# OpenDriveLab/ViDAR

Hardware: AMD Instinct MI355X
Metric: train samples/sec (6-cam->BEV step) (higher is better)
Workload: dtype f32

## Files before the change

### include/vidar_hip.h

```cpp
#ifndef VIDAR_HIP_H_
#define VIDAR_HIP_H_

#include <stddef.h>
#include <stdint.h>

#ifdef __cplusplus
extern "C" {
#endif

#define VIDAR_ERR_BAD_ARG (-22)

int vidar_abi_version(void);
int vidar_marker(int id, void* stream);

int vidar_set_deterministic(int on);
int vidar_get_deterministic(void);

int vidar_dvr_max_d(void);

int vidar_dvr_render_forward_f32(const float* sigma, const float* origin, const float* points,
                                 const float* tindex, float* pred_dist ,
                                 float* gt_dist , int N, int M, int T, int TO, int Z, int Y,
                                 int X, int train_phase, void* stream);

int vidar_dvr_render_f32(const float* sigma, const float* origin, const float* points,
                         const float* tindex, float* pred_dist, float* gt_dist, float* grad_sigma,
                         int N, int M, int T, int TO, int Z, int Y, int X, int loss_type,
                         void* stream);

int vidar_dvr_init_f32(const float* points, const float* tindex, float* occupancy, int N, int M,
                       int T, int Z, int Y, int X, void* stream);

int vidar_dvxlr_max_d(void);


int vidar_dvr_set_sort_min_waves(int min_waves);
int vidar_dvr_set_traversal(int mode);
int vidar_dvxlr_set_pad_mode(int mode);

int vidar_dvxlr_render_f32(const float* sigma, const float* origin, const float* points,
                           const float* tindex, float* pred_dist, float* gt_dist, float* dd_dsigma,
                           float* indices, int N, int M, int T, int TO, int Z, int Y, int X,
                           void* stream);

size_t vidar_dvxlr_get_grad_sigma_workspace_bytes(int N, int T, int Z, int Y, int X, int volumes );
int vidar_dvxlr_get_grad_sigma_f32(const float* elementwise_mult ,
                                   const float* indices , const float* tindex,
                                   float* grad_sigma , int N, int M, int L, int T,
                                   int Z, int Y, int X, void* workspace, size_t workspace_bytes,
                                   void* stream);

int vidar_dvxlr2_render_f32(const float* sigma, const float* origin, const float* points,
                            const float* tindex, const float* sigma_regul, float* pred_dist,
                            float* gt_dist, float* dd_dsigma, float* indices, float* ray_pred,
                            float* indicator, int N, int M, int T, int TO, int Z, int Y, int X,
                            void* stream);

int vidar_dvxlr2_get_grad_sigma_f32(const float* elementwise_mult, const float* indices,
                                    const float* tindex, const float* indicator,
                                    const float* grad_ray_pred, float* grad_sigma,
                                    float* grad_sigma_regul, int N, int M, int L, int T, int Z, int Y,
                                    int X, void* workspace, size_t workspace_bytes, void* stream);

size_t vidar_knn1_d3_workspace_bytes(int N, int P1);
int vidar_knn1_d3_fwd(const float* p1, const float* p2, const int64_t* lengths1,
                      const int64_t* lengths2, int64_t* idx, float* dist2, void* workspace, int N,
                      int P1, int P2, void* stream);
int vidar_knn1_d3_bwd(const float* p1, const float* p2, const int64_t* lengths1,
                      const int64_t* lengths2, const int64_t* idx, const float* grad_dist2,
                      float* grad_p1, float* grad_p2, int N, int P1, int P2, void* stream);
int vidar_knn1_d3_bwd_workspace_bytes(int N, int P2, int64_t* bytes);
int vidar_knn1_d3_bwd_ws(const float* p1, const float* p2, const int64_t* lengths1,
                         const int64_t* lengths2, const int64_t* idx, const float* grad_dist2,
                         float* grad_p1, float* grad_p2, int N, int P1, int P2, void* workspace,
                         size_t workspace_bytes, void* stream);

int vidar_msda_fwd_f32(const float* value, const int64_t* spatial_shapes,
                       const int64_t* level_start_index, const float* sampling_loc,
                       const float* attn_weight, float* out, int B, int Nv, int H, int C, int Nq,
                       int L, int P, void* stream);
size_t vidar_msda_bwd_workspace_bytes(int B, int Nv, int H, int Nq, int L, int P);
int vidar_msda_set_item_order(int head_major);
int vidar_msda_bwd_f32(const float* value, const int64_t* spatial_shapes,
                       const int64_t* level_start_index, const float* sampling_loc,
                       const float* attn_weight, const float* grad_out, float* grad_value,
                       float* grad_sampling_loc, float* grad_attn_weight, int B, int Nv, int H, int C,
                       int Nq, int L, int P, void* workspace, size_t workspace_bytes, void* stream);

int vidar_msda_fused_fwd_f32(const float* value, const int64_t* spatial_shapes,
                             const int64_t* level_start_index, const float* off_raw, const float* logit_raw,
                             const float* ref, float* loc_out, float* w_out, float* out, int bs, int Qn, int Nv,
                             int H, int C, int Nq, int L, int P, int R, int mode, int merge_queue, void* stream);
int vidar_msda_fused_bwd_f32(const float* value, const int64_t* spatial_shapes,
                             const int64_t* level_start_index, const float* sampling_loc,
                             const float* attn_weight, const float* grad_out, float* grad_value,
                             float* grad_off_raw, float* grad_logit_raw, int bs, int Qn, int Nv, int H, int C,
                             int Nq, int L, int P, int merge_queue, void* workspace, size_t workspace_bytes, void* stream);

int vidar_drop_add_ln_fwd_f32(const float* x, const float* residual, const float* gamma, const float* beta, float* y,
                              float* sum_out, float* mean_out, float* rstd_out, int64_t rows, int C, float p, float eps,
                              uint32_t seed, void* stream);
int vidar_drop_add_ln_bwd_f32(const float* grad_y, const float* sum_in, const float* gamma, const float* mean_in,
                              const float* rstd_in, float* grad_x, float* grad_residual, float* grad_gamma,
                              float* grad_beta, void* workspace, int64_t rows, int C, float p, uint32_t seed,
                              void* stream);
size_t vidar_drop_add_ln_bwd_workspace_bytes(int64_t rows);

int vidar_relu_drop_fwd_f32(const float* x, float* y, int64_t n, float p, uint32_t seed, void* stream);
int vidar_relu_drop_bwd_f32(const float* grad_y, const float* y, float* grad_x, int64_t n, float p, void* stream);

int vidar_colsum_f32(const float* x, float* out, int64_t rows, int cols, void* stream);

int vidar_sca_plan_f32(const float* ref_3d, const float* lidar2img, float* ref_cam, uint8_t* bev_mask,
                       float* count, int64_t* idx, uint8_t* valid, int32_t* lens, int32_t* slot_of,
                       const float* pc_range, float img_h, float img_w, int F, int B, int N, int Q, int D,
                       void* stream);
int vidar_sca_rows_f32(const float* src, const int64_t* idx, const uint8_t* valid, const float* count, float* dst,
                       int B, int N, int S, int stride, int Q, int C, void* stream);
int vidar_sca_combine_f32(const float* src, const int32_t* slot_of, const float* count, float* dst, int B, int N,
                          int S, int Q, int C, void* stream);

size_t vidar_latent_render_bwd_workspace_bytes(int bs, int H, int W, int Z, int maps );
int vidar_latent_render_prob_fwd_f32(const float* occ, float* path_prob, int bs, int H, int W, int Z,
                                     int grid_num, float step, int act, void* stream);
int vidar_latent_render_prob_bwd_f32(const float* occ, const float* grad_path_prob, float* grad_occ,
                                     int bs, int H, int W, int Z, int grid_num, float step, int act,
                                     void* workspace, size_t workspace_bytes, void* stream);
int vidar_latent_render_gather_fwd_f32(const float* path_prob, const float* lora_a, float* feat,
                                       float* msum, int bs, int H, int W, int Z, int grid_num,
                                       float step, float eps, void* stream);
int vidar_latent_render_gather_bwd_f32(const float* path_prob, const float* lora_a, const float* feat,
                                       const float* msum, const float* grad_feat,
                                       float* grad_path_prob, float* grad_lora_a, int bs, int H,
                                       int W, int Z, int grid_num, float step, float eps,
                                       void* workspace, size_t workspace_bytes, void* stream);
int vidar_latent_render_gather_grouped_fwd_f32(const float* path_prob, const float* lora_a, float* feat, float* msum,
                                               int bs, int H, int W, int Z, int A, int grid_num, float step,
                                               float eps, void* stream);
int vidar_latent_render_gather_grouped_bwd_f32(const float* path_prob, const float* lora_a, const float* feat,
                                               const float* msum, const float* grad_feat, float* grad_path_prob,
                                               float* grad_lora_a, int bs, int H, int W, int Z, int A, int grid_num,
                                               float step, float eps, void* workspace, size_t workspace_bytes,
                                               void* stream);

size_t vidar_ray_bwd_workspace_bytes(int F, int Z, int Y, int X);
int vidar_ray_ce_fwd_f32(const float* sigma, const float* origin, const float* gt_pts,
                         const float* tindex, float* ce, float* lse, float* valid, int F, int R,
                         int Z, int Y, int X, int K, float step, void* stream);
int vidar_ray_ce_bwd_f32(const float* sigma, const float* origin, const float* gt_pts,
                         const float* tindex, const float* lse, const float* grad_ce,
                         float* grad_sigma, int F, int R, int Z, int Y, int X, int K, float step,
                         void* workspace, size_t workspace_bytes, void* stream);
int vidar_ray_gumbel_fwd_f32(const float* sigma, const float* origin, const float* pts,
                             const float* tindex, const float* noise , float* dist,
                             float* aux , int F, int R, int Z, int Y, int X, int K,
                             float step, void* stream);
int vidar_ray_gumbel_bwd_f32(const float* sigma, const float* origin, const float* pts,
                             const float* tindex, const float* aux, const float* grad_dist,
                             float* grad_sigma, int F, int R, int Z, int Y, int X, int K, float step,
                             void* workspace, size_t workspace_bytes, void* stream);
int vidar_ray_argmax_f32(const float* sigma, const float* origin, const float* pts,
                         const float* tindex, float* pred_dist, float* gt_dist, int F, int R, int Z,
                         int Y, int X, int K, float step, void* stream);
int vidar_ray_dist_fwd_f32(const float* sigma, const float* origin, const float* gt_pts,
                           const float* tindex, const float* noise , float* dist,
                           float* gt_len, float* aux , float* valid, int F, int R, int Z,
                           int Y, int X, int K, float step, void* stream);
int vidar_ray_dist_bwd_f32(const float* sigma, const float* origin, const float* gt_pts,
                           const float* tindex, const float* aux, const float* grad_dist,
                           float* grad_sigma, int F, int R, int Z, int Y, int X, int K, float step,
                           void* workspace, size_t workspace_bytes, void* stream);
int vidar_ray_max_k(void);
int vidar_ray_force_streamed(int on);

#define VIDAR_GEMM_F32 0
#define VIDAR_GEMM_BF16X3 1
#define VIDAR_GEMM_K_MAJOR 0
#define VIDAR_GEMM_MN_MAJOR 1
int vidar_gemm_f32(const float* A, int64_t lda, int a_layout, const float* B, int64_t ldb, int b_layout, float* C,
                   int64_t ldc, int M, int N, int K, int batch, int64_t strideA, int64_t strideB, int64_t strideC,
                   const float* scale, const float* shift, int vec_axis, const float* residual, int64_t ldr,
                   int64_t strideR, int relu, int precision, int reduce, float* a_rowsum, void* workspace,
                   size_t workspace_bytes, void* stream);
int vidar_gemm_splits(int M, int N, int K, int batch, int precision, int reduce);
size_t vidar_gemm_workspace_bytes(int M, int N, int K, int batch, int precision, int reduce);
int vidar_gemm_set_variant(int variant);

int vidar_dcn_set_variant(int variant);
int vidar_dcn_im2col_f32(const float* x, const float* offset, const float* mask, float* cols, int N,
                         int C, int H, int W, int Ho, int Wo, int kh, int kw, int stride, int pad,
                         int dil, void* stream);
int vidar_dcn_col2im_det_workspace_bytes(int N, int C, int H, int W, int64_t* bytes);
int vidar_dcn_col2im_f32(const float* grad_cols, const float* x, const float* offset,
                         const float* mask, float* grad_x, float* grad_offset, float* grad_mask,
                         int N, int C, int H, int W, int Ho, int Wo, int kh, int kw, int stride,
                         int pad, int dil, void* workspace, size_t workspace_bytes, void* stream);
size_t vidar_dcn_col2im_workspace_bytes(int N, int H, int W, int Ho, int Wo, int kh, int kw);

size_t vidar_conv3x3_few_workspace_bytes(int C);
int vidar_conv3x3_few_f32(const float* x, const float* weight, const float* bias, float* out, int N, int C, int H, int W,
                          int Cout, void* workspace, size_t workspace_bytes, void* stream);

int vidar_affine_act_fwd_f32(const float* x, const float* scale, const float* shift,
                             const float* residual, float* y, int N, int C, int HW, int relu,
                             void* stream);
int vidar_stem_bn_relu_pool_f32(const float* x, const float* scale, const float* shift, float* y, int N, int C,
                                int H, int W, void* stream);
int vidar_affine_act_bwd_f32(const float* grad_y, const float* y, const float* scale, float* grad_x,
                             float* grad_residual, int N, int C, int HW, int relu, void* stream);

int vidar_dcnv3_set_variant(int variant);
int vidar_dcnv3_forward_f32(const float* input, const float* offset, const float* mask, float* out, int N, int H, int W,
                            int kh, int kw, int stride_h, int stride_w, int pad_h, int pad_w, int dil_h, int dil_w,
                            int group, int group_channels, float offset_scale, void* stream);
size_t vidar_dcnv3_backward_workspace_bytes(int N, int H, int W, int kh, int kw, int stride_h, int stride_w, int pad_h,
                                            int pad_w, int dil_h, int dil_w, int group, int group_channels);
int vidar_dcnv3_backward_f32(const float* input, const float* offset, const float* mask, const float* grad_out,
                             float* grad_input, float* grad_offset, float* grad_mask, int N, int H, int W, int kh, int kw,
                             int stride_h, int stride_w, int pad_h, int pad_w, int dil_h, int dil_w, int group,
                             int group_channels, float offset_scale, void* workspace, size_t workspace_bytes, void* stream);

int vidar_det_match_cost_f32(const float* cls, const float* box, const float* gt_box_norm, const int32_t* gt_label,
                             const int32_t* gt_start, float* cost, float alpha, float gamma, float cls_weight,
                             float reg_weight, int NL, int B, int Q, int C, int total_g, void* stream);
size_t vidar_det_loss_workspace_bytes(int NL, int B, int Q);
int vidar_det_loss_fwd_f32(const float* cls, const float* box, const int32_t* labels, const int32_t* matched_gt,
                           const float* gt_box_norm, const int32_t* gt_start, const float* code_weights, float* sums,
                           float alpha, float gamma, int NL, int B, int Q, int C, int total_g, void* workspace,
                           size_t workspace_bytes, void* stream);
int vidar_det_loss_bwd_f32(const float* cls, const float* box, const int32_t* labels, const int32_t* matched_gt,
                           const float* gt_box_norm, const int32_t* gt_start, const float* code_weights,
                           const float* grad_sums, float* grad_cls, float* grad_box, float alpha, float gamma, int NL,
                           int B, int Q, int C, int total_g, void* stream);

#define VIDAR_IMG_PHOTO_FLOATS 12
int vidar_img_photometric_u8(const uint8_t* src, const float* photo, uint8_t* dst, int n, int H, int W, void* stream);
int vidar_img_photometric_f32(const uint8_t* src, const float* photo, float* dst, int n, int H, int W, void* stream);
size_t vidar_img_resample_workspace_bytes(int n, int crop_h, int out_w);
int vidar_img_resample_u8(const uint8_t* src, uint8_t* dst, int n, int H, int W, int crop_x, int crop_y, int crop_w,
                          int crop_h, int out_w, int out_h, const int32_t* tab_x, int ksize_x, const int32_t* tab_y,
                          int ksize_y, int flip, void* workspace, size_t workspace_bytes, void* stream);
int vidar_img_normalise_f32(const uint8_t* src, const float* photo, float* dst, int n, int H, int W, int out_h, int out_w,
                            int Hp, int Wp, const float* mean, const float* stdv, int to_rgb, void* stream);

#ifdef __cplusplus
}
#endif
#endif
```

### vidar_amd/_lib.py

```python
from __future__ import annotations

import ctypes
import os
from pathlib import Path

_PKG = Path(__file__).resolve().parent
LIB_PATH = _PKG / "libvidar_hip.so"
_lib = None
BAD_ARG = -22


class VidarHipError(RuntimeError):
    pass


def lib() -> ctypes.CDLL:
    global _lib
    if _lib is None:
        import torch
        if not LIB_PATH.exists():
            raise VidarHipError(
                f"{LIB_PATH} not found: build it with `python -m vidar_amd.build` "
                f"(or __graft_entry__.build()); vidar_amd has no CPU fallback")
        _lib = declare(ctypes.CDLL(str(LIB_PATH)))
        dcn = os.environ.get("VIDAR_DCN_VARIANT")
        if dcn is not None:
            _lib.vidar_dcn_set_variant(int(dcn))
        v3 = os.environ.get("VIDAR_DCNV3_VARIANT")
        if v3 is not None:
            _lib.vidar_dcnv3_set_variant(int(v3))
        order = os.environ.get("VIDAR_MSDA_ITEM_ORDER")
        if order is not None:
            _lib.vidar_msda_set_item_order(int(order))
    return _lib


_KIND = {"p": ctypes.c_void_p, "i": ctypes.c_int, "l": ctypes.c_int64, "z": ctypes.c_size_t, "f": ctypes.c_float,
         "u": ctypes.c_uint32}
_ABI = {
    "vidar_abi_version": "i",
    "vidar_marker": "i i p",
    "vidar_set_deterministic": "i i",
    "vidar_get_deterministic": "i",
    "vidar_dvr_max_d": "i",
    "vidar_dvr_render_forward_f32": "i 6p 8i p",
    "vidar_dvr_render_f32": "i 7p 8i p",
    "vidar_dvr_init_f32": "i 3p 6i p",
    "vidar_dvxlr_max_d": "i",
    "vidar_dvr_set_sort_min_waves": "i i",
    "vidar_dvr_set_traversal": "i i",
    "vidar_dvxlr_set_pad_mode": "i i",
    "vidar_dvxlr_render_f32": "i 8p 7i p",
    "vidar_dvxlr_get_grad_sigma_workspace_bytes": "z 6i",
    "vidar_dvxlr_get_grad_sigma_f32": "i 4p 7i p z p",
    "vidar_dvxlr2_render_f32": "i 11p 7i p",
    "vidar_dvxlr2_get_grad_sigma_f32": "i 7p 7i p z p",
    "vidar_knn1_d3_workspace_bytes": "z 2i",
    "vidar_knn1_d3_fwd": "i 7p 3i p",
    "vidar_knn1_d3_bwd": "i 8p 3i p",
    "vidar_knn1_d3_bwd_workspace_bytes": "i 2i p",
    "vidar_knn1_d3_bwd_ws": "i 8p 3i p z p",
    "vidar_msda_fwd_f32": "i 6p 7i p",
    "vidar_msda_bwd_workspace_bytes": "z 6i",
    "vidar_msda_set_item_order": "i i",
    "vidar_msda_bwd_f32": "i 9p 7i p z p",
    "vidar_msda_fused_fwd_f32": "i 9p 11i p",
    "vidar_msda_fused_bwd_f32": "i 9p 9i p z p",
    "vidar_drop_add_ln_fwd_f32": "i 8p l i 2f u p",
    "vidar_drop_add_ln_bwd_f32": "i 10p l i f u p",
    "vidar_drop_add_ln_bwd_workspace_bytes": "z l",
    "vidar_relu_drop_fwd_f32": "i 2p l f u p",
    "vidar_relu_drop_bwd_f32": "i 3p l f p",
    "vidar_colsum_f32": "i 2p l i p",
    "vidar_sca_plan_f32": "i 10p 2f 5i p",
    "vidar_sca_rows_f32": "i 5p 6i p",
    "vidar_sca_combine_f32": "i 4p 5i p",
    "vidar_latent_render_bwd_workspace_bytes": "z 5i",
    "vidar_latent_render_prob_fwd_f32": "i 2p 5i f i p",
    "vidar_latent_render_prob_bwd_f32": "i 3p 5i f i p z p",
    "vidar_latent_render_gather_fwd_f32": "i 4p 5i 2f p",
    "vidar_latent_render_gather_bwd_f32": "i 7p 5i 2f p z p",
    "vidar_latent_render_gather_grouped_fwd_f32": "i 4p 6i 2f p",
    "vidar_latent_render_gather_grouped_bwd_f32": "i 7p 6i 2f p z p",
    "vidar_ray_bwd_workspace_bytes": "z 4i",
    "vidar_ray_ce_fwd_f32": "i 7p 6i f p",
    "vidar_ray_ce_bwd_f32": "i 7p 6i f p z p",
    "vidar_ray_gumbel_fwd_f32": "i 7p 6i f p",
    "vidar_ray_gumbel_bwd_f32": "i 7p 6i f p z p",
    "vidar_ray_argmax_f32": "i 6p 6i f p",
    "vidar_ray_dist_fwd_f32": "i 9p 6i f p",
    "vidar_ray_dist_bwd_f32": "i 7p 6i f p z p",
    "vidar_ray_max_k": "i",
    "vidar_ray_force_streamed": "i i",
    "vidar_gemm_f32": "i p l i p l i p l 4i 3l 2p i p 2l 3i 2p z p",
    "vidar_gemm_splits": "i 6i",
    "vidar_gemm_workspace_bytes": "z 6i",
    "vidar_gemm_set_variant": "i i",
    "vidar_dcn_set_variant": "i i",
    "vidar_dcn_im2col_f32": "i 4p 11i p",
    "vidar_dcn_col2im_f32": "i 7p 11i p z p",
    "vidar_dcn_col2im_workspace_bytes": "z 7i",
    "vidar_dcn_col2im_det_workspace_bytes": "i 4i p",
    "vidar_conv3x3_few_workspace_bytes": "z i",
    "vidar_conv3x3_few_f32": "i 4p 5i p z p",
    "vidar_affine_act_fwd_f32": "i 5p 4i p",
    "vidar_stem_bn_relu_pool_f32": "i 4p 4i p",
    "vidar_affine_act_bwd_f32": "i 5p 4i p",
    "vidar_dcnv3_set_variant": "i i",
    "vidar_dcnv3_forward_f32": "i 4p 13i f p",
    "vidar_dcnv3_backward_workspace_bytes": "z 13i",
    "vidar_dcnv3_backward_f32": "i 7p 13i f p z p",
    "vidar_det_match_cost_f32": "i 6p 4f 5i p",
    "vidar_det_loss_workspace_bytes": "z 3i",
    "vidar_det_loss_fwd_f32": "i 8p 2f 5i p z p",
    "vidar_det_loss_bwd_f32": "i 10p 2f 5i p",
    "vidar_img_photometric_u8": "i 3p 3i p",
    "vidar_img_photometric_f32": "i 3p 3i p",
    "vidar_img_resample_workspace_bytes": "z 3i",
    "vidar_img_resample_u8": "i 2p 9i p i p 2i p z p",
    "vidar_img_normalise_f32": "i 3p 7i 2p i p",
}


def signature(name):
    ret, *runs = _ABI[name].split()
    return _KIND[ret], [_KIND[r[-1]] for r in runs for _ in range(int(r[:-1] or 1))]


def declare(cdll):
    for name in _ABI:
        try:
            fn = getattr(cdll, name)
        except AttributeError:
            raise VidarHipError(f"{name} is not exported by {cdll._name}: rebuild the library") from None
        fn.restype, fn.argtypes = signature(name)
    return cdll


def check(rc: int, what: str):
    if rc == 0:
        return
    if rc == BAD_ARG:
        raise ValueError(f"{what}: invalid argument")
    raise VidarHipError(f"{what}: HIP error {rc}")


def ptr(t):
    return None if t is None else t.data_ptr()


def workspace(nbytes_fn, *dims, like):
    import torch
    n = nbytes_fn(*dims)
    if n == 0:
        return None, None, 0
    ws = torch.empty(n, dtype=torch.uint8, device=like.device)
    return ws, ptr(ws), n


def stream_of(t):
    import torch
    return torch.cuda.current_stream(t.device).cuda_stream


class OpTimer:
    def __init__(self):
        self.enabled = False
        self.records = {}

    def reset(self):
        self.records = {}

    class _Span:
        __slots__ = ("t", "name", "nbytes", "e0")

        def __init__(self, t, name, nbytes):
            self.t, self.name, self.nbytes = t, name, nbytes

        def __enter__(self):
            import torch
            self.e0 = torch.cuda.Event(enable_timing=True)
            self.e0.record()

        def __exit__(self, *exc):
            import torch
            e1 = torch.cuda.Event(enable_timing=True)
            e1.record()
            self.t.records.setdefault(self.name, []).append((self.e0, e1, self.nbytes))

    class _Null:
        def __enter__(self): return None
        def __exit__(self, *exc): return False

    _null = _Null()

    def span(self, name, nbytes=0):
        return OpTimer._Span(self, name, nbytes) if self.enabled else OpTimer._null

    def summary(self):
        import torch
        torch.cuda.synchronize()
        out = {}
        for name, recs in self.records.items():
            ms = [a.elapsed_time(b) for a, b, _ in recs]
            out[name] = dict(calls=len(ms), total_ms=sum(ms), avg_ms=sum(ms) / len(ms),
                             bytes_per_call=sum(r[2] for r in recs) / len(recs))
        return out


TIMER = OpTimer()
```

### vidar_amd/csrc/dcn.hip

```cpp
#include <hip/hip_runtime.h>
#include <stdint.h>

#include "vidar_hip.h"
#include "vidar_common.h"
#include "det_scatter.h"

namespace {

struct PlaneTile { int plane, tile; bool ok; };
__device__ __forceinline__ PlaneTile xcd_plane_tile(int L, int T, int planes) {
  const int xcd = L & 7, j = L >> 3;
  const int pl = (j / T) * 8 + xcd;
  return PlaneTile{pl, j - (j / T) * T, pl < planes};
}
inline unsigned xcd_plane_grid(int T, int planes) { return 8u * (unsigned)T * (unsigned)((planes + 7) / 8); }

struct Conv { int C, H, W, Ho, Wo, kh, kw, stride, pad, dil; };

struct Bil {
  int h0, w0;
  float lh, lw;
  bool in, t, b, l, r;
};

__device__ __forceinline__ Bil bil(float h, float w, int H, int W) {
  Bil q;
  q.in = h > -1.f && w > -1.f && h < H && w < W;
  q.h0 = (int)floorf(h); q.w0 = (int)floorf(w);
  q.lh = h - q.h0; q.lw = w - q.w0;
  q.t = q.h0 >= 0; q.b = q.h0 + 1 <= H - 1; q.l = q.w0 >= 0; q.r = q.w0 + 1 <= W - 1;
  return q;
}

struct Pos { float h, w; };
__device__ __forceinline__ Pos tap_pos(const Conv& g, int py, int px, int t, float oh, float ow) {
  const int i = t / g.kw, j = t - i * g.kw;
  return Pos{py * g.stride - g.pad + i * g.dil + oh, px * g.stride - g.pad + j * g.dil + ow};
}

template <class F>
__device__ __forceinline__ void for_corners(const Bil& q, int W, F f) {
  const float hh = 1.f - q.lh, hw = 1.f - q.lw;
  const int tl = q.h0 * W + q.w0;
  if (q.t && q.l) f(tl, hh * hw);
  if (q.t && q.r) f(tl + 1, hh * q.lw);
  if (q.b && q.l) f(tl + W, q.lh * hw);
  if (q.b && q.r) f(tl + W + 1, q.lh * q.lw);
}

constexpr int kMaxTaps = 9;

typedef float pair_t __attribute__((ext_vector_type(2), aligned(4)));

template <bool PAIR>
__device__ __forceinline__ pair_t load_pair(const void* p) {
  if constexpr (PAIR) return *reinterpret_cast<const pair_t*>(p);
  else return pair_t{*reinterpret_cast<const float*>(p), 0.f};
}

struct PairMap {
  int top, bot;
  bool same, left;
  __device__ __forceinline__ float e0(float cl, float cr) const { return same ? cl : (left ? cr : 0.f); }
  __device__ __forceinline__ float e1(float cl, float cr) const { return same ? cr : (left ? 0.f : cl); }
};

__device__ __forceinline__ PairMap pair_map(const Bil& q, int H, int W) {
  const int c0 = min(max(q.w0, 0), max(W - 2, 0));
  const int r0 = min(max(q.h0, 0), H - 1), r1 = min(max(q.h0 + 1, 0), H - 1);
  return PairMap{r0 * W + c0, r1 * W + c0, q.w0 == c0, q.w0 < c0};
}

constexpr int kCP = 16;
struct TapFoot { unsigned top, bot; float wt0, wt1, wb0, wb1; };

__device__ __forceinline__ TapFoot tap_foot(Pos s, float m, const Conv& g) {
  const Bil q = bil(s.h, s.w, g.H, g.W);
  const PairMap pm = pair_map(q, g.H, g.W);
  const float wl = (q.l ? 1.f - q.lw : 0.f), wr = (q.r ? q.lw : 0.f);
  const float a0 = pm.e0(wl, wr), a1 = pm.e1(wl, wr);
  const float ht = (q.t ? 1.f - q.lh : 0.f) * m, hb = (q.b ? q.lh : 0.f) * m;
  TapFoot f;
  f.top = (unsigned)pm.top * 4u; f.bot = (unsigned)pm.bot * 4u;
  f.wt0 = q.in ? ht * a0 : 0.f; f.wt1 = q.in ? ht * a1 : 0.f;
  f.wb0 = q.in ? hb * a0 : 0.f; f.wb1 = q.in ? hb * a1 : 0.f;
  return f;
}

template <bool PAIR>
__device__ __forceinline__ void im2col_body(const float* __restrict__ x, const float* __restrict__ offset,
                                            const float* __restrict__ mask, float* __restrict__ cols, const Conv& g, int nimg) {
  const int P = g.Ho * g.Wo, K = g.kh * g.kw;
  const int cgroups = (g.C + kCP - 1) / kCP;
  const PlaneTile pt = xcd_plane_tile(blockIdx.x, (P + 255) / 256, cgroups * nimg);
  if (!pt.ok) return;
  const int p = pt.tile * 256 + threadIdx.x;
  if (p >= P) return;
  const int n = pt.plane / cgroups, c0 = (pt.plane - n * cgroups) * kCP, nc = min(kCP, g.C - c0);
  const int py = p / g.Wo, px = p % g.Wo;
  const size_t plane = (size_t)g.H * g.W, KP = (size_t)K * P;
  const char* im = reinterpret_cast<const char*>(x + ((size_t)n * g.C + c0) * plane);
  float* out = cols + ((size_t)n * g.C + c0) * KP + p;
  const float* off_n = offset + (size_t)n * 2 * K * P + p;
  const float* msk_n = mask + (size_t)n * K * P + p;
  float oh = off_n[0], ow = off_n[P], m = msk_n[0];
  for (int t = 0; t < K; ++t) {
    const TapFoot f = tap_foot(tap_pos(g, py, px, t, oh, ow), m, g);
    pair_t a[kCP], b[kCP];
#pragma unroll
    for (int c = 0; c < kCP; ++c) {
      const char* pl = im + (size_t)(c < nc ? c : 0) * plane * 4;
      a[c] = load_pair<PAIR>(pl + f.top);
      b[c] = load_pair<PAIR>(pl + f.bot);
    }
    if (t + 1 < K) {
      oh = off_n[(size_t)(2 * t + 2) * P]; ow = off_n[(size_t)(2 * t + 3) * P]; m = msk_n[(size_t)(t + 1) * P];
    }
#pragma unroll
    for (int c = 0; c < kCP; ++c)
      if (c < nc) {
        const float v = f.wt0 * a[c].x + f.wt1 * a[c].y + f.wb0 * b[c].x + f.wb1 * b[c].y;
        __builtin_nontemporal_store(v, out + (size_t)c * KP + (size_t)t * P);
      }
  }
}

__global__ __launch_bounds__(256) void dcn_im2col_pair_kernel(
    const float* __restrict__ x, const float* __restrict__ offset, const float* __restrict__ mask,
    float* __restrict__ cols, Conv g, int nimg) {
  im2col_body<true>(x, offset, mask, cols, g, nimg);
}
__global__ __launch_bounds__(256) void dcn_im2col_kernel(
    const float* __restrict__ x, const float* __restrict__ offset, const float* __restrict__ mask,
    float* __restrict__ cols, Conv g, int nimg) {
  im2col_body<false>(x, offset, mask, cols, g, nimg);
}

constexpr int kCG = 8;
template <class Acc, class... AccParam>
__global__ __launch_bounds__(256) void dcn_col2im_kernel(const float* __restrict__ grad_cols, const float* __restrict__ offset,
                                                         const float* __restrict__ mask, float* __restrict__ grad_x, Conv g,
                                                         AccParam... acc_param) {
  Acc acc(grad_x, acc_param...);
  const int P = g.Ho * g.Wo, K = g.kh * g.kw;
  const int p = blockIdx.x * 256 + threadIdx.x;
  if constexpr (!Acc::kMeasureOnly) {
    if (p >= P) return;
  }
  const int n = blockIdx.z, c0 = blockIdx.y * kCG, nc = min(kCG, g.C - c0);
  const int py = p / g.Wo, px = p % g.Wo;
  const size_t plane = (size_t)g.H * g.W, KP = (size_t)K * P;
  float* gim = grad_x + ((size_t)n * g.C + c0) * plane;
  const float* gc = grad_cols + ((size_t)n * g.C + c0) * KP + p;
  for (int t = 0; t < K; ++t) {
    if constexpr (Acc::kMeasureOnly) {
      if (p >= P) break;
    }
    const size_t o = ((size_t)n * 2 * K + 2 * t) * P + p;
    const Pos s = tap_pos(g, py, px, t, offset[o], offset[o + P]);
    const Bil q = bil(s.h, s.w, g.H, g.W);
    if (!q.in) continue;
    const float m = mask[((size_t)n * K + t) * P + p];
    for (int c = 0; c < nc; ++c) {
      const float gv = gc[(size_t)c * KP + (size_t)t * P] * m;
      if (gv == 0.f) continue;
      for_corners(q, g.W, [&](int pix, float w) { acc.add(gim + (size_t)c * plane + pix, w * gv); });
    }
  }
  if constexpr (Acc::kMeasureOnly) acc.flush();
}

struct Entry { int src; float w; };

template <bool FILL>
__global__ __launch_bounds__(256) void dcn_revmap_kernel(const float* __restrict__ offset,
                                                         const float* __restrict__ mask, int* __restrict__ cursor,
                                                         Entry* __restrict__ rec, Conv g) {
  const int P = g.Ho * g.Wo, K = g.kh * g.kw, HW = g.H * g.W;
  const int p = blockIdx.x * 256 + threadIdx.x;
  if (p >= P) return;
  const int t = blockIdx.y, n = blockIdx.z;
  const int py = p / g.Wo, px = p % g.Wo;
  const size_t o = ((size_t)n * 2 * K + 2 * t) * P + p;
  const Pos s = tap_pos(g, py, px, t, offset[o], offset[o + P]);
  const Bil q = bil(s.h, s.w, g.H, g.W);
  if (!q.in) return;
  const float m = FILL ? mask[((size_t)n * K + t) * P + p] : 0.f;
  int* cur = cursor + ((size_t)n * K + t) * HW;
  const int src = t * P + p;
  for_corners(q, g.W, [&](int pix, float w) {
    if (FILL) rec[atomicAdd(cur + pix, 1)] = Entry{src, w * m};
    else atomicAdd(cur + pix, 1);
  });
}

__global__ __launch_bounds__(1024) void dcn_revmap_scan_kernel(int* __restrict__ cursor, int* __restrict__ first,
                                                               int HW, int per_image) {
  __shared__ int s_part[1024];
  const int n = blockIdx.x;
  int* cnt = cursor + (size_t)n * HW;
  int* fst = first + (size_t)n * HW;
  const int per = (HW + 1023) / 1024;
  const int r0 = min(HW, (int)threadIdx.x * per), r1 = min(HW, r0 + per);
  int sum = 0;
  for (int i = r0; i < r1; ++i) sum += cnt[i];
  s_part[threadIdx.x] = sum;
  __syncthreads();
  for (int d = 1; d < 1024; d <<= 1) {
    const int a = (int)threadIdx.x >= d ? s_part[threadIdx.x - d] : 0;
    __syncthreads();
    s_part[threadIdx.x] += a;
    __syncthreads();
  }
  int run = n * per_image + s_part[threadIdx.x] - sum;
  for (int i = r0; i < r1; ++i) { const int c = cnt[i]; fst[i] = run; cnt[i] = run; run += c; }
}

constexpr int kGC = 16;
__global__ __launch_bounds__(256) void dcn_col2im_gather_kernel(const float* __restrict__ grad_cols,
                                                                const int* __restrict__ first,
                                                                const int* __restrict__ last,
                                                                const Entry* __restrict__ rec,
                                                                float* __restrict__ grad_x, Conv g) {
  const int P = g.Ho * g.Wo, K = g.kh * g.kw, HW = g.H * g.W;
  const int pix = blockIdx.x * 256 + threadIdx.x;
  if (pix >= HW) return;
  const int n = blockIdx.z, c0 = blockIdx.y * kGC;
  float acc[kGC];
#pragma unroll
  for (int c = 0; c < kGC; ++c) acc[c] = 0.f;
  const size_t KP = (size_t)K * P;
  const float* gc = grad_cols + ((size_t)n * g.C + c0) * KP;
  const int nc = min(kGC, g.C - c0);
  for (int t = 0; t < K; ++t) {
    const size_t bin = ((size_t)n * K + t) * HW + pix;
    const int e0 = first[bin], e1 = last[bin];
    if (nc == kGC) {
      int e = e0;
      for (; e + 1 < e1; e += 2) {
        const Entry r0 = rec[e], r1 = rec[e + 1];
        float v0[kGC], v1[kGC];
#pragma unroll
        for (int c = 0; c < kGC; ++c) { v0[c] = gc[(size_t)c * KP + r0.src]; v1[c] = gc[(size_t)c * KP + r1.src]; }
#pragma unroll
        for (int c = 0; c < kGC; ++c) acc[c] += r0.w * v0[c] + r1.w * v1[c];
      }
      if (e < e1) {
        const Entry r = rec[e];
#pragma unroll
        for (int c = 0; c < kGC; ++c) acc[c] += r.w * gc[(size_t)c * KP + r.src];
      }
    } else {
      for (int e = e0; e < e1; ++e) {
        const Entry r = rec[e];
        for (int c = 0; c < nc; ++c) acc[c] += r.w * gc[(size_t)c * KP + r.src];
      }
    }
  }
  for (int c = 0; c < nc; ++c) grad_x[((size_t)n * g.C + c0 + c) * HW + pix] = acc[c];
}

#ifndef VIDAR_DCN_GRY
#define VIDAR_DCN_GRY 2
#endif
#ifndef VIDAR_DCN_GLC
#define VIDAR_DCN_GLC 8
#endif
constexpr int kGRY = VIDAR_DCN_GRY;
constexpr int kGTH = 8 * kGRY, kGTW = 32;
#ifndef VIDAR_DCN_GHALO
#define VIDAR_DCN_GHALO 5
#endif
constexpr int kGHalo = VIDAR_DCN_GHALO;
constexpr int kGWH = kGTH + 2 * kGHalo + 2;
constexpr int kGWW = kGTW + 2 * kGHalo + 2;
constexpr int kGWP = (kGWW + 3) / 4 * 4;
constexpr int kGWS = kGWH * kGWP;
constexpr int kGLC = VIDAR_DCN_GLC;
constexpr int kGPos = (kGWS + 255) / 256;

__global__ __launch_bounds__(256) void dcn_col2im_gather_lds_kernel(
    const float* __restrict__ grad_cols, const int* __restrict__ first, const int* __restrict__ last,
    const Entry* __restrict__ rec, float* __restrict__ grad_x, Conv g, int tiles_x, int tiles_y, int nimg, float inv_wo) {
  __shared__ __attribute__((aligned(16))) float s_gc[kGLC * kGWS];
  constexpr int K = 9;
  const int P = g.Ho * g.Wo, HW = g.H * g.W;
  const int cgroups = (g.C + kGLC - 1) / kGLC;
  const PlaneTile pt = xcd_plane_tile(blockIdx.x, tiles_x * tiles_y, cgroups * nimg);
  if (!pt.ok) return;
  const int tile = pt.tile, tyi = tile / tiles_x, txi = tile - tyi * tiles_x;
  const int n = pt.plane / cgroups, c0 = (pt.plane - n * cgroups) * kGLC, nc = min(kGLC, g.C - c0);
  const int ry = threadIdx.x / kGTW, rx = threadIdx.x % kGTW;
  const int dx = txi * kGTW + rx;
  const size_t KP = (size_t)K * P;
  const float* gc = grad_cols + ((size_t)n * g.C + c0) * KP;
  float acc[kGRY][kGLC];
#pragma unroll
  for (int k = 0; k < kGRY; ++k)
#pragma unroll
    for (int c = 0; c < kGLC; ++c) acc[k][c] = 0.f;
  for (int t = 0; t < K; ++t) {
    const int i = t / 3, j = t - i * 3;
    const int wy0 = tyi * kGTH + g.pad - i - kGHalo - 1, wx0 = txi * kGTW + g.pad - j - kGHalo - 1;
    const float* gct = gc + (size_t)t * P;
    __syncthreads();
    {
      const int wave = __builtin_amdgcn_readfirstlane((int)threadIdx.x >> 6);
#pragma unroll
      for (int k = 0; k < kGPos; ++k) {
        const int e = threadIdx.x + k * 256;
        const int r = e / kGWP, cc = e - r * kGWP;
        const int sy = wy0 + r, sx = wx0 + cc;
        const bool ok = e < kGWS && sy >= 0 && sy < g.Ho && sx >= 0 && sx < g.Wo && cc < kGWW;
        const int off = ok ? sy * g.Wo + sx : 0;
        if (ok) {
#pragma unroll
          for (int c = 0; c < kGLC; ++c)
            __builtin_amdgcn_global_load_lds((const __attribute__((address_space(1))) void*)(gct + (size_t)(c < nc ? c : 0) * KP + off),
                                             (__attribute__((address_space(3))) void*)(s_gc + c * kGWS + k * 256 + wave * 64), 4, 0, 0);
        }
      }
    }
    __syncthreads();
    if (dx >= g.W) continue;
#pragma unroll
    for (int k = 0; k < kGRY; ++k) {
      const int dy = tyi * kGTH + ry + 8 * k;
      if (dy >= g.H) continue;
      const size_t bin = ((size_t)n * K + t) * HW + dy * g.W + dx;
      const int e1 = last[bin];
      int e = first[bin];
      Entry nxt = e < e1 ? rec[e] : Entry{0, 0.f};
      while (e < e1) {
        const Entry r = nxt;
        ++e;
        if (e < e1) nxt = rec[e];
        const int p = r.src - t * P;
        const int py = (int)((p + 0.5f) * inv_wo), px = p - py * g.Wo;
        const int ly = py - wy0, lx = px - wx0;
        if (ly >= 0 && ly < kGWH && lx >= 0 && lx < kGWW) {
          const float* q = s_gc + ly * kGWP + lx;
#pragma unroll
          for (int c = 0; c < kGLC; ++c) acc[k][c] += r.w * q[c * kGWS];
        } else {
          for (int c = 0; c < nc; ++c) acc[k][c] += r.w * gct[(size_t)c * KP + p];
        }
      }
    }
  }
  if (dx < g.W) {
#pragma unroll
    for (int k = 0; k < kGRY; ++k) {
      const int dy = tyi * kGTH + ry + 8 * k;
      if (dy < g.H)
        for (int c = 0; c < nc; ++c) grad_x[((size_t)n * g.C + c0 + c) * HW + dy * g.W + dx] = acc[k][c];
    }
  }
}

int g_dcn_variant = 1;

template <bool PAIR>
__device__ __forceinline__ void col2im_coord_body(const float* __restrict__ grad_cols, const float* __restrict__ x,
                                                  const float* __restrict__ offset, const float* __restrict__ mask,
                                                  float* __restrict__ grad_offset, float* __restrict__ grad_mask,
                                                  const Conv& g) {
  const int P = g.Ho * g.Wo, K = g.kh * g.kw;
  const int p = blockIdx.x * 256 + threadIdx.x;
  if (p >= P) return;
  const int t = blockIdx.y, n = blockIdx.z;
  const int py = p / g.Wo, px = p % g.Wo;
  const size_t o = ((size_t)n * 2 * K + 2 * t) * P + p;
  const Pos s = tap_pos(g, py, px, t, offset[o], offset[o + P]);
  const float m = mask[((size_t)n * K + t) * P + p];
  const Bil q = bil(s.h, s.w, g.H, g.W);
  float gh = 0.f, gw = 0.f, gm = 0.f;
  if (q.in) {
    const float hh = 1.f - q.lh, hw = 1.f - q.lw;
    const PairMap pm = pair_map(q, g.H, g.W);
    const float tl = (q.t && q.l) ? 1.f : 0.f, tr = (q.t && q.r) ? 1.f : 0.f;
    const float bl = (q.b && q.l) ? 1.f : 0.f, br = (q.b && q.r) ? 1.f : 0.f;
    const float m_t0 = pm.e0(hh * hw * tl, hh * q.lw * tr), m_t1 = pm.e1(hh * hw * tl, hh * q.lw * tr);
    const float m_b0 = pm.e0(q.lh * hw * bl, q.lh * q.lw * br), m_b1 = pm.e1(q.lh * hw * bl, q.lh * q.lw * br);
    const float h_t0 = pm.e0(-hw * tl, -q.lw * tr), h_t1 = pm.e1(-hw * tl, -q.lw * tr);
    const float h_b0 = pm.e0(hw * bl, q.lw * br), h_b1 = pm.e1(hw * bl, q.lw * br);
    const float w_t0 = pm.e0(-hh * tl, hh * tr), w_t1 = pm.e1(-hh * tl, hh * tr);
    const float w_b0 = pm.e0(-q.lh * bl, q.lh * br), w_b1 = pm.e1(-q.lh * bl, q.lh * br);
    int c = 0;
    constexpr int kCB = 8;
    const unsigned top_b = (unsigned)pm.top * 4u, bot_b = (unsigned)pm.bot * 4u, p_b = (unsigned)p * 4u;
    const size_t plane_b = (size_t)g.H * g.W * 4, col_b = (size_t)K * P * 4;
    for (; c + kCB <= g.C; c += kCB) {
      const char* im0 = reinterpret_cast<const char*>(x) + ((size_t)n * g.C + c) * plane_b;
      const char* gc0 = reinterpret_cast<const char*>(grad_cols) + (((size_t)n * g.C + c) * K + t) * (size_t)P * 4;
      pair_t a[kCB], b[kCB];
      float gc[kCB];
#pragma unroll
      for (int u = 0; u < kCB; ++u) {
        gc[u] = *reinterpret_cast<const float*>(gc0 + u * col_b + p_b);
        a[u] = load_pair<PAIR>(im0 + u * plane_b + top_b);
        b[u] = load_pair<PAIR>(im0 + u * plane_b + bot_b);
      }
      __builtin_amdgcn_sched_barrier(0);
#pragma unroll
      for (int u = 0; u < kCB; ++u) {
        gm += gc[u] * (m_t0 * a[u].x + m_t1 * a[u].y + m_b0 * b[u].x + m_b1 * b[u].y);
        gh += gc[u] * (h_t0 * a[u].x + h_t1 * a[u].y + h_b0 * b[u].x + h_b1 * b[u].y);
        gw += gc[u] * (w_t0 * a[u].x + w_t1 * a[u].y + w_b0 * b[u].x + w_b1 * b[u].y);
      }
    }
    for (; c < g.C; ++c) {
      const float* im = x + ((size_t)n * g.C + c) * g.H * g.W;
      const float gc = grad_cols[(((size_t)n * g.C + c) * K + t) * P + p];
      const pair_t a = load_pair<PAIR>(im + pm.top), b = load_pair<PAIR>(im + pm.bot);
      gm += gc * (m_t0 * a.x + m_t1 * a.y + m_b0 * b.x + m_b1 * b.y);
      gh += gc * (h_t0 * a.x + h_t1 * a.y + h_b0 * b.x + h_b1 * b.y);
      gw += gc * (w_t0 * a.x + w_t1 * a.y + w_b0 * b.x + w_b1 * b.y);
    }
  }
  grad_offset[o] = gh * m;
  grad_offset[o + P] = gw * m;
  grad_mask[((size_t)n * K + t) * P + p] = gm;
}

__global__ __launch_bounds__(256) void dcn_col2im_coord_kernel(
    const float* __restrict__ grad_cols, const float* __restrict__ x, const float* __restrict__ offset,
    const float* __restrict__ mask, float* __restrict__ grad_offset, float* __restrict__ grad_mask, Conv g) {
  col2im_coord_body<true>(grad_cols, x, offset, mask, grad_offset, grad_mask, g);
}
__global__ __launch_bounds__(256) void dcn_col2im_coord_1col_kernel(
    const float* __restrict__ grad_cols, const float* __restrict__ x, const float* __restrict__ offset,
    const float* __restrict__ mask, float* __restrict__ grad_offset, float* __restrict__ grad_mask, Conv g) {
  col2im_coord_body<false>(grad_cols, x, offset, mask, grad_offset, grad_mask, g);
}

inline bool dcn_bad(int N, const Conv& g) {
  return N < 0 || g.C <= 0 || g.H <= 0 || g.W <= 0 || g.Ho <= 0 || g.Wo <= 0 || g.kh <= 0 ||
         g.kw <= 0 || g.stride <= 0 || g.dil <= 0 || g.pad < 0;
}

}

extern "C" {

int vidar_dcn_set_variant(int variant) {
  const int prev = g_dcn_variant;
  if (variant >= 0 && variant <= 1) g_dcn_variant = variant;
  return prev;
}

int vidar_dcn_im2col_f32(const float* x, const float* offset, const float* mask, float* cols, int N,
                         int C, int H, int W, int Ho, int Wo, int kh, int kw, int stride, int pad,
                         int dil, void* stream) {
  VIDAR_ENTER();
  Conv g{C, H, W, Ho, Wo, kh, kw, stride, pad, dil};
  if (dcn_bad(N, g)) return VIDAR_ERR_BAD_ARG;
  if (N == 0) return 0;
  if (kh * kw > kMaxTaps) return VIDAR_ERR_BAD_ARG;
  hipLaunchKernelGGL(W >= 2 ? dcn_im2col_pair_kernel : dcn_im2col_kernel,
                     dim3(xcd_plane_grid((Ho * Wo + 255) / 256, ((C + kCP - 1) / kCP) * N)), dim3(256), 0, (hipStream_t)stream,
                     x, offset, mask, cols, g, N);
  return vidar_last_error();
}

size_t vidar_dcn_col2im_workspace_bytes(int N, int H, int W, int Ho, int Wo, int kh, int kw) {
  if (N <= 0 || H <= 0 || W <= 0 || Ho <= 0 || Wo <= 0 || kh <= 0 || kw <= 0) return 0;
  const size_t hw = (size_t)N * kh * kw * H * W, ent = (size_t)N * kh * kw * Ho * Wo * 4;
  if (ent >= (1ull << 31)) return 0;
  return sizeof(int) * 2 * hw + sizeof(Entry) * ent;
}

int vidar_dcn_col2im_det_workspace_bytes(int N, int C, int H, int W, int64_t* bytes) {
  if (N < 0 || C < 0 || H < 0 || W < 0 || !bytes) return VIDAR_ERR_BAD_ARG;
  *bytes = (int64_t)det_workspace_bytes((size_t)N * C * H * W);
  return 0;
}

int vidar_dcn_col2im_f32(const float* grad_cols, const float* x, const float* offset,
                         const float* mask, float* grad_x, float* grad_offset, float* grad_mask,
                         int N, int C, int H, int W, int Ho, int Wo, int kh, int kw, int stride,
                         int pad, int dil, void* workspace, size_t workspace_bytes, void* stream) {
  VIDAR_ENTER();
  Conv g{C, H, W, Ho, Wo, kh, kw, stride, pad, dil};
  if (dcn_bad(N, g)) return VIDAR_ERR_BAD_ARG;
  hipStream_t s = (hipStream_t)stream;
  if (N == 0) return 0;
  if (kh * kw > kMaxTaps) return VIDAR_ERR_BAD_ARG;
  const int P = Ho * Wo, K = kh * kw, HW = H * W;
  if (det_mode()) {
    const dim3 grid((P + 255) / 256, (C + kCG - 1) / kCG, N);
    const int rc = det_scatter(
        grad_x, nullptr, (size_t)N * C * HW, 0, (uint64_t)N * C * K * P * 4, false, workspace, workspace_bytes, s,
        [&](uint32_t* word, uint32_t*) {
          hipLaunchKernelGGL((dcn_col2im_kernel<det::AccMeasure, det::AccMeasure::Param>), grid, dim3(256), 0, s, grad_cols, offset, mask, grad_x, g,
                             det::AccMeasure::Param{word});
        },
        [&](long long* acc, long long*, const uint32_t* word, const uint32_t*, int h) {
          hipLaunchKernelGGL((dcn_col2im_kernel<det::AccFixed, det::AccFixed::Param>), grid, dim3(256), 0, s, grad_cols, offset, mask, grad_x, g,
                             det::AccFixed::Param{acc, word, h});
        });
    if (rc != 0) return rc;
  } else if (workspace) {
    const size_t need = vidar_dcn_col2im_workspace_bytes(N, H, W, Ho, Wo, kh, kw);
    if (need == 0 || workspace_bytes < need) return VIDAR_ERR_BAD_ARG;
    int* cursor = (int*)workspace;
    int* first = cursor + (size_t)N * K * HW;
    Entry* rec = (Entry*)(first + (size_t)N * K * HW);
    hipError_t e = hipMemsetAsync(cursor, 0, sizeof(int) * (size_t)N * K * HW, s);
    if (e != hipSuccess) return (int)e;
    const dim3 rgrid((P + 255) / 256, K, N);
    hipLaunchKernelGGL(dcn_revmap_kernel<false>, rgrid, dim3(256), 0, s, offset, mask, cursor, rec, g);
    hipLaunchKernelGGL(dcn_revmap_scan_kernel, dim3(N * K), dim3(1024), 0, s, cursor, first, HW, P * 4);
    hipLaunchKernelGGL(dcn_revmap_kernel<true>, rgrid, dim3(256), 0, s, offset, mask, cursor, rec, g);
    if ((g_dcn_variant & 1) && kh == 3 && kw == 3 && stride == 1 && dil == 1 && Ho == H && Wo == W) {
      const int tiles_x = (W + kGTW - 1) / kGTW, tiles_y = (H + kGTH - 1) / kGTH;
      hipLaunchKernelGGL(dcn_col2im_gather_lds_kernel, dim3(xcd_plane_grid(tiles_x * tiles_y, ((C + kGLC - 1) / kGLC) * N)), dim3(256), 0,
                         s, grad_cols, first, cursor, rec, grad_x, g, tiles_x, tiles_y, N, 1.0f / (float)Wo);
    } else {
      hipLaunchKernelGGL(dcn_col2im_gather_kernel, dim3((HW + 255) / 256, (C + kGC - 1) / kGC, N), dim3(256), 0, s,
                         grad_cols, first, cursor, rec, grad_x, g);
    }
  } else {
    hipError_t e = hipMemsetAsync(grad_x, 0, sizeof(float) * (size_t)N * C * H * W, s);
    if (e != hipSuccess) return (int)e;
    hipLaunchKernelGGL(dcn_col2im_kernel<det::AccAtomic>, dim3((P + 255) / 256, (C + kCG - 1) / kCG, N), dim3(256), 0, s, grad_cols,
                       offset, mask, grad_x, g);
  }
  hipLaunchKernelGGL(W >= 2 ? dcn_col2im_coord_kernel : dcn_col2im_coord_1col_kernel, dim3((P + 255) / 256, K, N), dim3(256), 0,
                     s, grad_cols, x, offset, mask, grad_offset, grad_mask, g);
  return vidar_last_error();
}

}
```

### vidar_amd/plugin/backbones.py

```python
from __future__ import annotations

import ctypes
import math
import os

import torch
import torch.nn as nn
import torch.nn.functional as F
from torch.autograd import Function
from torch.autograd.function import once_differentiable

from .registry import BACKBONES, NECKS
from .._lib import lib, check, ptr, stream_of, workspace, TIMER
from .. import gemm as G
from .. import deterministic


def dcn_col2im(grad_cols, x, offset, mask, kh, kw, stride, pad, dil, Ho, Wo, gather=True):
    N, C, H, W = x.shape
    gx = torch.empty_like(x); goff = torch.empty_like(offset); gm = torch.empty_like(mask)
    if deterministic.sync():
        nbytes = ctypes.c_int64(0)
        check(lib().vidar_dcn_col2im_det_workspace_bytes(N, C, H, W, ctypes.addressof(nbytes)), "dcn_col2im")
        nbytes = nbytes.value
        ws = torch.empty(nbytes, dtype=torch.uint8, device=x.device)
        ws_ptr = ptr(ws)
    else:
        ws, ws_ptr, nbytes = workspace(lib().vidar_dcn_col2im_workspace_bytes, N, H, W, Ho, Wo, kh, kw, like=x) \
            if gather else (None, None, 0)
    with TIMER.span("dcn_col2im", 4 * (3 * x.numel() + 2 * offset.numel() + 2 * mask.numel() + grad_cols.numel())):
        check(lib().vidar_dcn_col2im_f32(ptr(grad_cols), ptr(x), ptr(offset), ptr(mask), ptr(gx), ptr(goff), ptr(gm),
                                         N, C, H, W, Ho, Wo, kh, kw, stride, pad, dil, ws_ptr, nbytes, stream_of(x)),
              "dcn_col2im")
    return gx, goff, gm


class _ModulatedDeformConv(Function):

    @staticmethod
    def forward(ctx, x, offset, mask, weight, bias, stride, pad, dil, gemm_mode="lib", scale=None, shift=None,
                relu=False):
        x, offset, mask = x.float().contiguous(), offset.float().contiguous(), mask.float().contiguous()
        N, C, H, W = x.shape
        Cout, _, kh, kw = weight.shape
        Ho = (H + 2 * pad - dil * (kh - 1) - 1) // stride + 1
        Wo = (W + 2 * pad - dil * (kw - 1) - 1) // stride + 1
        cols = torch.empty((N, C * kh * kw, Ho * Wo), device=x.device)
        with TIMER.span("dcn_im2col", 4 * (x.numel() + offset.numel() + mask.numel() + cols.numel())):
            check(lib().vidar_dcn_im2col_f32(ptr(x), ptr(offset), ptr(mask), ptr(cols), N, C, H, W, Ho,
                                             Wo, kh, kw, stride, pad, dil, stream_of(x)), "dcn_im2col")
        fused = scale is not None
        if gemm_mode == "lib":
            assert not fused
            out = torch.bmm(weight.reshape(1, Cout, -1).expand(N, -1, -1), cols)
            if bias is not None:
                out = out + bias.view(1, -1, 1)
        else:
            sh = shift
            if bias is not None:
                sh = bias.float() if not fused else (shift + bias.float() * scale)
            out = G.conv_forward(weight.reshape(Cout, -1), cols, scale, sh, None, relu, G.precision_of(gemm_mode))
        ctx.save_for_backward(x, offset, mask, weight, cols, scale, out if (fused and relu) else None)
        ctx.cfg = (stride, pad, dil, Ho, Wo, bias is not None, gemm_mode, fused, relu)
        return out.view(N, Cout, Ho, Wo)

    @staticmethod
    @once_differentiable
    def backward(ctx, grad_out):
        x, offset, mask, weight, cols, scale, y = ctx.saved_tensors
        stride, pad, dil, Ho, Wo, has_bias, gemm_mode, fused, relu = ctx.cfg
        N, C, H, W = x.shape
        Cout, _, kh, kw = weight.shape
        go = grad_out.float().contiguous().view(N, Cout, Ho * Wo)
        if fused:
            go = _affine_act_backward(go, y if relu else go, scale, relu, False)[0]
        if gemm_mode == "lib":
            grad_weight = torch.bmm(go, cols.transpose(1, 2)).sum(0).reshape(weight.shape)
            grad_cols = torch.bmm(weight.reshape(1, Cout, -1).transpose(1, 2).expand(N, -1, -1), go)
        else:
            prec = G.precision_of(gemm_mode)
            grad_weight = G.conv_grad_weight(go, cols, prec).reshape(weight.shape) if ctx.needs_input_grad[3] else None
            grad_cols = G.conv_grad_input(weight.reshape(Cout, -1), go, prec)
        gx, goff, gm = dcn_col2im(grad_cols, x, offset, mask, kh, kw, stride, pad, dil, Ho, Wo)
        return (gx, goff, gm, grad_weight, (go.sum((0, 2)) if has_bias else None), None, None, None, None, None, None,
                None)


def modulated_deform_conv2d(x, offset, mask, weight, bias=None, stride=1, padding=0, dilation=1, bn=None, relu=False):
    m = G.mode() if (x.is_cuda and G.own_kernels()) else "lib"
    scale = shift = None
    if bn is not None:
        assert m != "lib"
        scale, shift = bn._scale_shift()
    return _ModulatedDeformConv.apply(x, offset, mask, weight, bias, int(stride), int(padding), int(dilation), m,
                                      scale, shift, bool(relu))


_CONV_OFFSET_OWN = os.environ.get("VIDAR_CONV_OFFSET", "lib") == "own"


class _Conv3x3Few(Function):

    @staticmethod
    def forward(ctx, x, weight, bias):
        x = x.contiguous()
        w = weight.contiguous()
        N, C, H, W = x.shape
        Cout = w.shape[0]
        out = torch.empty((N, Cout, H, W), device=x.device, dtype=torch.float32)
        ws, ws_ptr, ws_bytes = workspace(lib().vidar_conv3x3_few_workspace_bytes, C, like=x)
        with TIMER.span("conv3x3_few", 4 * (x.numel() + out.numel())):
            check(lib().vidar_conv3x3_few_f32(ptr(x), ptr(w), ptr(bias), ptr(out), N, C, H, W, Cout, ws_ptr, ws_bytes,
                                              stream_of(x)), "conv3x3_few")
        ctx.save_for_backward(x, w)
        ctx.has_bias = bias is not None
        return out

    @staticmethod
    @once_differentiable
    def backward(ctx, g):
        x, w = ctx.saved_tensors
        need = [ctx.needs_input_grad[0], ctx.needs_input_grad[1], ctx.has_bias and ctx.needs_input_grad[2]]
        gx, gw, gb = torch.ops.aten.convolution_backward(g.contiguous(), x, w, [w.shape[0]] if ctx.has_bias else None,
                                                         [1, 1], [1, 1], [1, 1], False, [0, 0], 1, need)
        return gx, gw, gb


def conv3x3_few_ok(conv, x):
    return (_CONV_OFFSET_OWN and x.is_cuda and x.dtype == torch.float32 and conv.weight.dtype == torch.float32
            and not torch.is_autocast_enabled() and x.dim() == 4
            and conv.kernel_size == (3, 3) and conv.stride == (1, 1) and conv.padding == (1, 1) and conv.dilation == (1, 1)
            and conv.groups == 1 and conv.padding_mode == "zeros" and conv.out_channels <= 32 and conv.in_channels % 8 == 0
            and x.shape[3] <= 191 and x.shape[2] * x.shape[3] < (1 << 30) and x.numel() > 0)


class ModulatedDeformConv2dPack(nn.Module):

    def __init__(self, in_channels, out_channels, kernel_size, stride=1, padding=0, dilation=1,
                 groups=1, deform_groups=1, bias=True):
        super().__init__()
        if groups != 1 or deform_groups != 1:
            raise NotImplementedError("DCNv2 kernels are built for groups == deform_groups == 1")
        k = kernel_size
        self.stride, self.padding, self.dilation, self.k = stride, padding, dilation, k
        self.weight = nn.Parameter(torch.empty(out_channels, in_channels, k, k))
        self.bias = nn.Parameter(torch.zeros(out_channels)) if bias else None
        n = in_channels * k * k
        nn.init.uniform_(self.weight, -1.0 / math.sqrt(n), 1.0 / math.sqrt(n))
        self.conv_offset = nn.Conv2d(in_channels, 3 * k * k, k, stride, padding, dilation, bias=True)
        nn.init.zeros_(self.conv_offset.weight)
        nn.init.zeros_(self.conv_offset.bias)

    def forward(self, x, bn=None, relu=False):
        if conv3x3_few_ok(self.conv_offset, x):
            out = _Conv3x3Few.apply(x, self.conv_offset.weight, self.conv_offset.bias)
        else:
            out = self.conv_offset(x)
        o1, o2, mask = torch.chunk(out, 3, dim=1)
        offset = torch.cat((o1, o2), dim=1)
        fuse = dict(bn=bn, relu=relu) if bn is not None else {}
        return modulated_deform_conv2d(x, offset, torch.sigmoid(mask), self.weight, self.bias,
                                       self.stride, self.padding, self.dilation, **fuse)


class _AffineAct(Function):

    @staticmethod
    def forward(ctx, x, scale, shift, residual, relu):
        x = x.float().contiguous()
        N, C, H, W = x.shape
        res = residual.float().contiguous() if residual is not None else None
        y = torch.empty_like(x)
        with TIMER.span("affine_act_fwd", 4 * x.numel() * (3 if res is not None else 2)):
            check(lib().vidar_affine_act_fwd_f32(ptr(x), ptr(scale), ptr(shift), ptr(res), ptr(y), N, C,
                                                 H * W, int(relu), stream_of(x)), "affine_act_fwd")
        ctx.save_for_backward(y, scale)
        ctx.cfg = (relu, residual is not None)
        return y

    @staticmethod
    @once_differentiable
    def backward(ctx, gy):
        y, scale = ctx.saved_tensors
        relu, has_res = ctx.cfg
        gx, gres = _affine_act_backward(gy.float().contiguous(), y, scale, relu, has_res)
        return gx, None, None, gres, None


def _affine_act_backward(gy, y, scale, relu, has_res):
    N, C = y.shape[:2]
    HW = y.numel() // (N * C)
    gx = torch.empty_like(y)
    gres = torch.empty_like(y) if has_res else None
    with TIMER.span("affine_act_bwd", 4 * y.numel() * (4 if has_res else 3)):
        check(lib().vidar_affine_act_bwd_f32(ptr(gy), ptr(y), ptr(scale), ptr(gx), ptr(gres), N, C,
                                             HW, int(relu), stream_of(y)), "affine_act_bwd")
    return gx, gres


class FrozenBN(nn.BatchNorm2d):

    def __init__(self, c, requires_grad=False):
        super().__init__(c)
        for p in self.parameters():
            p.requires_grad = requires_grad
        self._cache = None

    def _scale_shift(self):
        key = (self.weight._version, self.bias._version, self.running_mean._version,
               self.running_var._version, self.weight.device)
        if self._cache is None or self._cache[0] != key:
            with torch.no_grad():
                scale = (self.weight / torch.sqrt(self.running_var + self.eps)).float().contiguous()
                shift = (self.bias - self.running_mean * scale).float().contiguous()
            self._cache = (key, scale, shift)
        return self._cache[1], self._cache[2]

    def forward(self, x, residual=None, relu=False):
        if self.weight.requires_grad or not x.is_cuda:
            y = F.batch_norm(x, self.running_mean, self.running_var, self.weight, self.bias, False, 0.0,
                             self.eps)
            if residual is not None:
                y = y + residual
            return F.relu(y, inplace=True) if relu else y
        scale, shift = self._scale_shift()
        return _AffineAct.apply(x, scale, shift, residual, relu)


def stem_bn_relu_pool(x, bn):
    if not x.is_cuda or bn.weight.requires_grad or (torch.is_grad_enabled() and x.requires_grad):
        return None
    x = x.float().contiguous()
    N, C, H, W = x.shape
    if W % 4 or N * C > 65535:
        return None
    scale, shift = bn._scale_shift()
    y = torch.empty((N, C, (H - 1) // 2 + 1, W // 2), device=x.device, dtype=torch.float32)
    with TIMER.span("stem_bn_relu_pool", 4 * (x.numel() + y.numel())):
        check(lib().vidar_stem_bn_relu_pool_f32(ptr(x), ptr(scale), ptr(shift), ptr(y), N, C, H, W, stream_of(x)),
              "stem_bn_relu_pool")
    return y


class Conv1x1(nn.Conv2d):
    as_gemm = os.environ.get("VIDAR_CONV1X1_GEMM", "1") != "0"
    any_device = False

    def gemm_form(self, x):
        return (self.as_gemm and (x.is_cuda or self.any_device) and self.kernel_size == (1, 1) and self.padding == (0, 0)
                and self.groups == 1)

    def forward(self, x, presampled=False):
        if not self.gemm_form(x):
            assert not presampled
            return super().forward(x)
        if self.stride != (1, 1) and not presampled:
            x = x[:, :, ::self.stride[0], ::self.stride[1]].contiguous()
        N, C, H, W = x.shape
        out = torch.bmm(self.weight.view(1, self.out_channels, C).expand(N, -1, -1), x.reshape(N, C, H * W))
        if self.bias is not None:
            out = out + self.bias.view(1, -1, 1)
        return out.view(N, self.out_channels, H, W)


_AUTO_FUSE_RES = os.environ.get("VIDAR_AUTO_FUSE_RES", "1") != "0"


class _Conv1x1Identity(Function):

    @staticmethod
    def forward(ctx, x, weight):
        N, C, H, W = x.shape
        Cout = weight.shape[0]
        out = torch.bmm(weight.view(1, Cout, C).expand(N, -1, -1), x.reshape(N, C, H * W))
        ctx.save_for_backward(x, weight)
        return out.view(N, Cout, H, W), x.view_as(x)

    @staticmethod
    @once_differentiable
    def backward(ctx, g_out, g_ident):
        x, weight = ctx.saved_tensors
        N, C, H, W = x.shape
        Cout = weight.shape[0]
        gx = gw = None
        if g_out is None:
            return g_ident, None
        go = g_out.contiguous().view(N, Cout, H * W)
        if ctx.needs_input_grad[0]:
            wt = weight.view(1, Cout, C).transpose(1, 2).expand(N, -1, -1)
            if g_ident is not None:
                gx = g_ident.contiguous().view(N, C, H * W).baddbmm_(wt, go).view(N, C, H, W)
            else:
                gx = torch.bmm(wt, go).view(N, C, H, W)
        if ctx.needs_input_grad[1]:
            gw = torch.bmm(go, x.reshape(N, C, H * W).transpose(1, 2)).sum(0).view_as(weight)
        return gx, gw


_SHORTCUT_ACCUMULATE = os.environ.get("VIDAR_SHORTCUT_ACCUMULATE", "1") != "0"


def conv1x1_with_identity_ok(conv, x):
    return (_SHORTCUT_ACCUMULATE and isinstance(conv, Conv1x1) and conv.gemm_form(x) and conv.stride == (1, 1)
            and conv.bias is None and x.dtype == torch.float32 and conv.weight.dtype == torch.float32
            and x.requires_grad and torch.is_grad_enabled() and not torch.is_autocast_enabled() and x.is_contiguous())


class _Conv1x1BNAct(Function):

    @staticmethod
    def forward(ctx, x, weight, scale, shift, residual, relu, precision):
        x = x.float().contiguous()
        N, C, H, W = x.shape
        Cout = weight.shape[0]
        res = residual.float().contiguous().view(N, Cout, H * W) if residual is not None else None
        y = G.conv_forward(weight.reshape(Cout, C), x.view(N, C, H * W), scale, shift, res, relu, precision)
        ctx.save_for_backward(x, weight, scale, y if relu else None)
        ctx.cfg = (relu, residual is not None, precision)
        return y.view(N, Cout, H, W)

    @staticmethod
    @once_differentiable
    def backward(ctx, gy):
        x, weight, scale, y = ctx.saved_tensors
        relu, has_res, precision = ctx.cfg
        N, C, H, W = x.shape
        Cout = weight.shape[0]
        gy = gy.float().contiguous().view(N, Cout, H * W)
        gz, gres = _affine_act_backward(gy, y if relu else gy, scale, relu, has_res)
        gx = G.conv_grad_input(weight.reshape(Cout, C), gz, precision).view(N, C, H, W) if ctx.needs_input_grad[0] else None
        gw = G.conv_grad_weight(gz, x.view(N, C, H * W), precision).view_as(weight) if ctx.needs_input_grad[1] else None
        return gx, gw, None, None, (gres.view(N, Cout, H, W) if has_res else None), None, None


def _fuses_1x1(conv, bn, x, residual, hw, m):
    fuse = G.own_kernels(m) or (m == "auto" and residual is not None and _AUTO_FUSE_RES)
    in_range = 0 < hw < (1 << 22) and max(conv.in_channels, conv.out_channels) * hw < (1 << 29)
    return (fuse and x.is_cuda and not bn.weight.requires_grad and conv.bias is None and conv.kernel_size == (1, 1)
            and conv.padding == (0, 0) and conv.groups == 1 and in_range)


def conv1x1_bn_act(conv, bn, x, residual=None, relu=False, presampled=False):
    if presampled:
        return _conv1x1_bn_act_presampled(conv, bn, x, residual, relu)
    m = G.mode()
    hw = ((x.shape[2] - 1) // conv.stride[0] + 1) * ((x.shape[3] - 1) // conv.stride[1] + 1) if x.dim() == 4 else 0
    if not _fuses_1x1(conv, bn, x, residual, hw, m):
        return bn(conv(x), residual=residual, relu=relu)
    if conv.stride != (1, 1):
        x = x[:, :, ::conv.stride[0], ::conv.stride[1]]
    scale, shift = bn._scale_shift()
    return _Conv1x1BNAct.apply(x, conv.weight, scale, shift, residual, bool(relu), G.precision_of(m))


def _conv1x1_bn_act_presampled(conv, bn, xs, residual, relu):
    m = G.mode()
    if not _fuses_1x1(conv, bn, xs, residual, xs.shape[2] * xs.shape[3] if xs.dim() == 4 else 0, m):
        return bn(conv(xs, presampled=True), residual=residual, relu=relu)
    scale, shift = bn._scale_shift()
    return _Conv1x1BNAct.apply(xs, conv.weight, scale, shift, residual, bool(relu), G.precision_of(m))


_SHARE_SUBSAMPLE = os.environ.get("VIDAR_SHARE_SUBSAMPLE", "1") != "0"


class Bottleneck(nn.Module):
    expansion = 4

    def __init__(self, inplanes, planes, stride=1, downsample=None, style="caffe", dcn=None, bn_grad=False):
        super().__init__()
        s1, s2 = (stride, 1) if style == "caffe" else (1, stride)
        self.conv1 = Conv1x1(inplanes, planes, 1, stride=s1, bias=False)
        self.bn1 = FrozenBN(planes, bn_grad)
        if dcn is not None:
            self.conv2 = ModulatedDeformConv2dPack(planes, planes, 3, stride=s2, padding=1, dilation=1,
                                                   deform_groups=dcn.get("deform_groups", 1), bias=False)
        else:
            self.conv2 = nn.Conv2d(planes, planes, 3, stride=s2, padding=1, bias=False)
        self.bn2 = FrozenBN(planes, bn_grad)
        self.conv3 = Conv1x1(planes, planes * 4, 1, bias=False)
        self.bn3 = FrozenBN(planes * 4, bn_grad)
        self.downsample = downsample

    def _shares_subsample(self, x):
        d = self.downsample
        return (_SHARE_SUBSAMPLE and d is not None and len(d) == 2 and isinstance(d[0], Conv1x1) and isinstance(d[1], FrozenBN)
                and self.conv1.stride != (1, 1) and d[0].stride == self.conv1.stride
                and self.conv1.gemm_form(x) and d[0].gemm_form(x))

    def forward(self, x):
        if self._shares_subsample(x):
            sh, sw = self.conv1.stride
            xs = x[:, :, ::sh, ::sw].contiguous()
            identity = conv1x1_bn_act(self.downsample[0], self.downsample[1], xs, presampled=True)
            out = conv1x1_bn_act(self.conv1, self.bn1, xs, relu=True, presampled=True)
            return self._tail(out, identity)
        if self.downsample is None:
            identity = x
            if conv1x1_with_identity_ok(self.conv1, x) and not _fuses_1x1(self.conv1, self.bn1, x, None,
                                                                            x.shape[2] * x.shape[3], G.mode()):
                out, identity = _Conv1x1Identity.apply(x, self.conv1.weight)
                return self._tail(self.bn1(out, relu=True), identity)
        elif len(self.downsample) == 2 and isinstance(self.downsample[1], FrozenBN):
            identity = conv1x1_bn_act(self.downsample[0], self.downsample[1], x)
        else:
            identity = self.downsample(x)
        out = conv1x1_bn_act(self.conv1, self.bn1, x, relu=True)
        return self._tail(out, identity)

    def _tail(self, out, identity):
        if (isinstance(self.conv2, ModulatedDeformConv2dPack) and G.own_kernels() and out.is_cuda
                and not self.bn2.weight.requires_grad):
            out = self.conv2(out, bn=self.bn2, relu=True)
        else:
            out = self.bn2(self.conv2(out), relu=True)
        return conv1x1_bn_act(self.conv3, self.bn3, out, residual=identity, relu=True)


@BACKBONES.register_module()
class ResNet(nn.Module):
    arch = {50: (3, 4, 6, 3), 101: (3, 4, 23, 3), 152: (3, 8, 36, 3)}

    def __init__(self, depth=101, num_stages=4, out_indices=(0, 1, 2, 3), frozen_stages=-1,
                 norm_cfg=dict(type="BN", requires_grad=True), norm_eval=True, style="pytorch", dcn=None,
                 stage_with_dcn=(False, False, False, False), strides=(1, 2, 2, 2), in_channels=3,
                 base_channels=64, init_cfg=None, pretrained=None, **kwargs):
        super().__init__()
        if dcn is not None and dcn.get("type") != "DCNv2":
            raise NotImplementedError(dcn)
        bn_grad = norm_cfg.get("requires_grad", True)
        self.out_indices, self.frozen_stages, self.norm_eval = out_indices, frozen_stages, norm_eval
        self.conv1 = nn.Conv2d(in_channels, base_channels, 7, stride=2, padding=3, bias=False)
        self.bn1 = FrozenBN(base_channels, bn_grad)
        inplanes = base_channels
        self.res_layers = []
        for i, nblocks in enumerate(self.arch[depth][:num_stages]):
            planes = base_channels * 2 ** i
            stage_dcn = dcn if stage_with_dcn[i] else None
            down = None
            if strides[i] != 1 or inplanes != planes * 4:
                down = nn.Sequential(Conv1x1(inplanes, planes * 4, 1, stride=strides[i], bias=False),
                                     FrozenBN(planes * 4, bn_grad))
            blocks = [Bottleneck(inplanes, planes, strides[i], down, style, stage_dcn, bn_grad)]
            inplanes = planes * 4
            blocks += [Bottleneck(inplanes, planes, 1, None, style, stage_dcn, bn_grad) for _ in range(1, nblocks)]
            name = f"layer{i + 1}"
            self.add_module(name, nn.Sequential(*blocks))
            self.res_layers.append(name)
        self._freeze_stages()

    def _freeze_stages(self):
        if self.frozen_stages >= 0:
            for m in (self.conv1, self.bn1):
                for p in m.parameters():
                    p.requires_grad = False
        for i in range(1, self.frozen_stages + 1):
            for p in getattr(self, f"layer{i}").parameters():
                p.requires_grad = False

    def forward(self, x):
        x = self.conv1(x)
        y = stem_bn_relu_pool(x, self.bn1)
        x = y if y is not None else F.max_pool2d(self.bn1(x, relu=True), 3, stride=2, padding=1)
        outs = []
        for i, name in enumerate(self.res_layers):
            x = getattr(self, name)(x)
            if i in self.out_indices:
                outs.append(x)
        return tuple(outs)


class _ConvModule(nn.Module):

    def __init__(self, cin, cout, k, stride=1, padding=0):
        super().__init__()
        self.conv = nn.Conv2d(cin, cout, k, stride=stride, padding=padding)
        nn.init.xavier_uniform_(self.conv.weight)
        nn.init.zeros_(self.conv.bias)

    def forward(self, x):
        return self.conv(x)


@NECKS.register_module()
class FPN(nn.Module):
    def __init__(self, in_channels, out_channels, num_outs, start_level=0, end_level=-1,
                 add_extra_convs=False, relu_before_extra_convs=False, init_cfg=None, **kwargs):
        super().__init__()
        self.start_level = start_level
        self.backbone_end_level = len(in_channels) if end_level == -1 else end_level
        self.num_outs = num_outs
        self.add_extra_convs = "on_input" if add_extra_convs is True else add_extra_convs
        self.relu_before_extra_convs = relu_before_extra_convs
        self.lateral_convs = nn.ModuleList()
        self.fpn_convs = nn.ModuleList()
        for i in range(start_level, self.backbone_end_level):
            self.lateral_convs.append(_ConvModule(in_channels[i], out_channels, 1))
            self.fpn_convs.append(_ConvModule(out_channels, out_channels, 3, padding=1))
        extra = num_outs - (self.backbone_end_level - start_level)
        if self.add_extra_convs and extra >= 1:
            for i in range(extra):
                cin = in_channels[self.backbone_end_level - 1] if (i == 0 and self.add_extra_convs == "on_input") else out_channels
                self.fpn_convs.append(_ConvModule(cin, out_channels, 3, stride=2, padding=1))

    def forward(self, inputs):
        lat = [l(inputs[i + self.start_level]) for i, l in enumerate(self.lateral_convs)]
        for i in range(len(lat) - 1, 0, -1):
            lat[i - 1] = lat[i - 1] + F.interpolate(lat[i], size=lat[i - 1].shape[2:], mode="nearest")
        outs = [self.fpn_convs[i](lat[i]) for i in range(len(lat))]
        if self.num_outs > len(outs):
            if not self.add_extra_convs:
                for _ in range(self.num_outs - len(outs)):
                    outs.append(F.max_pool2d(outs[-1], 1, stride=2))
            else:
                if self.add_extra_convs == "on_input":
                    src = inputs[self.backbone_end_level - 1]
                elif self.add_extra_convs == "on_lateral":
                    src = lat[-1]
                else:
                    src = outs[-1]
                outs.append(self.fpn_convs[len(lat)](src))
                for i in range(len(lat) + 1, self.num_outs):
                    outs.append(self.fpn_convs[i](F.relu(outs[-1]) if self.relu_before_extra_convs else outs[-1]))
        return tuple(outs)
```

Measured before the change: 2.937.

## Fuse DCN offset chunk/cat/sigmoid into raw-offset im2col and col2im kernels

Adds RAW variants of the DCN im2col, col2im and coordinate-gradient kernels. They read the un-split offset-conv output directly, add the offset bias and apply the mask sigmoid in-kernel, and write the gradient for the raw tensor including the sigmoid derivative. A new _DeformConvPack autograd node replaces the chunk, cat, sigmoid and separate bias ops with these kernels. Its backward seeds the gather col2im accumulator with the offset conv's input gradient, which removes an extra add pass. This cuts several elementwise kernels and intermediate tensors per DCN layer, at the cost of recomputing expf on every tap access and a more complex backward ordering.

```diff
diff --git a/include/vidar_hip.h b/include/vidar_hip.h
--- a/include/vidar_hip.h
+++ b/include/vidar_hip.h
@@ -196,6 +196,13 @@
                          int N, int C, int H, int W, int Ho, int Wo, int kh, int kw, int stride,
                          int pad, int dil, void* workspace, size_t workspace_bytes, void* stream);
 size_t vidar_dcn_col2im_workspace_bytes(int N, int H, int W, int Ho, int Wo, int kh, int kw);
+int vidar_dcn_im2col_raw_f32(const float* x, const float* raw, const float* raw_bias, float* cols, int N,
+                             int C, int H, int W, int Ho, int Wo, int kh, int kw, int stride, int pad,
+                             int dil, void* stream);
+int vidar_dcn_col2im_raw_f32(const float* grad_cols, const float* x, const float* raw, const float* raw_bias,
+                             float* grad_x, const float* grad_x_base, float* grad_raw, int N, int C, int H, int W,
+                             int Ho, int Wo, int kh, int kw, int stride, int pad, int dil, void* workspace,
+                             size_t workspace_bytes, void* stream);
 
 size_t vidar_conv3x3_few_workspace_bytes(int C);
 int vidar_conv3x3_few_f32(const float* x, const float* weight, const float* bias, float* out, int N, int C, int H, int W,
diff --git a/vidar_amd/_lib.py b/vidar_amd/_lib.py
--- a/vidar_amd/_lib.py
+++ b/vidar_amd/_lib.py
@@ -101,6 +101,8 @@
     "vidar_dcn_col2im_f32": "i 7p 11i p z p",
     "vidar_dcn_col2im_workspace_bytes": "z 7i",
     "vidar_dcn_col2im_det_workspace_bytes": "i 4i p",
+    "vidar_dcn_im2col_raw_f32": "i 4p 11i p",
+    "vidar_dcn_col2im_raw_f32": "i 7p 11i p z p",
     "vidar_conv3x3_few_workspace_bytes": "z i",
     "vidar_conv3x3_few_f32": "i 4p 5i p z p",
     "vidar_affine_act_fwd_f32": "i 5p 4i p",
diff --git a/vidar_amd/csrc/dcn.hip b/vidar_amd/csrc/dcn.hip
--- a/vidar_amd/csrc/dcn.hip
+++ b/vidar_amd/csrc/dcn.hip
@@ -36,6 +36,37 @@
 __device__ __forceinline__ Pos tap_pos(const Conv& g, int py, int px, int t, float oh, float ow) {
   const int i = t / g.kw, j = t - i * g.kw;
   return Pos{py * g.stride - g.pad + i * g.dil + oh, px * g.stride - g.pad + j * g.dil + ow};
+}
+
+struct Tap { float oh, ow, m; };
+template <bool RAW>
+struct tap_index {
+  static __device__ __forceinline__ size_t off(int n, int t, int p, int K, int P) {
+    return ((size_t)n * (RAW ? 3 : 2) * K + 2 * t) * P + p;
+  }
+  static __device__ __forceinline__ size_t msk(int n, int t, int p, int K, int P) {
+    return ((size_t)n * (RAW ? 3 : 1) * K + (RAW ? 2 * K : 0) + t) * P + p;
+  }
+};
+template <bool RAW>
+__device__ __forceinline__ Tap load_tap(const float* __restrict__ offset, const float* __restrict__ mask, int n, int t, int p,
+                                        int K, int P) {
+  const size_t o = tap_index<RAW>::off(n, t, p, K, P);
+  return Tap{offset[o], offset[o + P], (RAW ? offset : mask)[tap_index<RAW>::msk(n, t, p, K, P)]};
+}
+template <bool RAW>
+__device__ __forceinline__ Tap activate(Tap v, const float* __restrict__ bias, int t, int K) {
+  if constexpr (RAW) {
+    v.oh += bias ? bias[2 * t] : 0.f;
+    v.ow += bias ? bias[2 * t + 1] : 0.f;
+    v.m = 1.f / (1.f + expf(-(v.m + (bias ? bias[2 * K + t] : 0.f))));
+  }
+  return v;
+}
+template <bool RAW>
+__device__ __forceinline__ Tap tap_operands(const float* __restrict__ offset, const float* __restrict__ mask,
+                                            const float* __restrict__ bias, int n, int t, int p, int K, int P) {
+  return activate<RAW>(load_tap<RAW>(offset, mask, n, t, p, K, P), bias, t, K);
 }
 
 template <class F>
@@ -87,9 +118,10 @@
   return f;
 }
 
-template <bool PAIR>
+template <bool PAIR, bool RAW>
 __device__ __forceinline__ void im2col_body(const float* __restrict__ x, const float* __restrict__ offset,
-                                            const float* __restrict__ mask, float* __restrict__ cols, const Conv& g, int nimg) {
+                                            const float* __restrict__ mask, const float* __restrict__ bias,
+                                            float* __restrict__ cols, const Conv& g, int nimg) {
   const int P = g.Ho * g.Wo, K = g.kh * g.kw;
   const int cgroups = (g.C + kCP - 1) / kCP;
   const PlaneTile pt = xcd_plane_tile(blockIdx.x, (P + 255) / 256, cgroups * nimg);
@@ -101,11 +133,10 @@
   const size_t plane = (size_t)g.H * g.W, KP = (size_t)K * P;
   const char* im = reinterpret_cast<const char*>(x + ((size_t)n * g.C + c0) * plane);
   float* out = cols + ((size_t)n * g.C + c0) * KP + p;
-  const float* off_n = offset + (size_t)n * 2 * K * P + p;
-  const float* msk_n = mask + (size_t)n * K * P + p;
-  float oh = off_n[0], ow = off_n[P], m = msk_n[0];
+  Tap nxt = load_tap<RAW>(offset, mask, n, 0, p, K, P);
   for (int t = 0; t < K; ++t) {
-    const TapFoot f = tap_foot(tap_pos(g, py, px, t, oh, ow), m, g);
+    const Tap op = activate<RAW>(nxt, bias, t, K);
+    const TapFoot f = tap_foot(tap_pos(g, py, px, t, op.oh, op.ow), op.m, g);
     pair_t a[kCP], b[kCP];
 #pragma unroll
     for (int c = 0; c < kCP; ++c) {
@@ -113,9 +144,7 @@
       a[c] = load_pair<PAIR>(pl + f.top);
       b[c] = load_pair<PAIR>(pl + f.bot);
     }
-    if (t + 1 < K) {
-      oh = off_n[(size_t)(2 * t + 2) * P]; ow = off_n[(size_t)(2 * t + 3) * P]; m = msk_n[(size_t)(t + 1) * P];
-    }
+    if (t + 1 < K) nxt = load_tap<RAW>(offset, mask, n, t + 1, p, K, P);
 #pragma unroll
     for (int c = 0; c < kCP; ++c)
       if (c < nc) {
@@ -128,19 +157,25 @@
 __global__ __launch_bounds__(256) void dcn_im2col_pair_kernel(
     const float* __restrict__ x, const float* __restrict__ offset, const float* __restrict__ mask,
     float* __restrict__ cols, Conv g, int nimg) {
-  im2col_body<true>(x, offset, mask, cols, g, nimg);
+  im2col_body<true, false>(x, offset, mask, nullptr, cols, g, nimg);
 }
 __global__ __launch_bounds__(256) void dcn_im2col_kernel(
     const float* __restrict__ x, const float* __restrict__ offset, const float* __restrict__ mask,
     float* __restrict__ cols, Conv g, int nimg) {
-  im2col_body<false>(x, offset, mask, cols, g, nimg);
+  im2col_body<false, false>(x, offset, mask, nullptr, cols, g, nimg);
+}
+template <bool PAIR>
+__global__ __launch_bounds__(256) void dcn_im2col_raw_kernel(
+    const float* __restrict__ x, const float* __restrict__ raw, const float* __restrict__ bias, float* __restrict__ cols,
+    Conv g, int nimg) {
+  im2col_body<PAIR, true>(x, raw, nullptr, bias, cols, g, nimg);
 }
 
 constexpr int kCG = 8;
-template <class Acc, class... AccParam>
+template <class Acc, bool RAW, class... AccParam>
 __global__ __launch_bounds__(256) void dcn_col2im_kernel(const float* __restrict__ grad_cols, const float* __restrict__ offset,
-                                                         const float* __restrict__ mask, float* __restrict__ grad_x, Conv g,
-                                                         AccParam... acc_param) {
+                                                         const float* __restrict__ mask, const float* __restrict__ bias,
+                                                         float* __restrict__ grad_x, Conv g, AccParam... acc_param) {
   Acc acc(grad_x, acc_param...);
   const int P = g.Ho * g.Wo, K = g.kh * g.kw;
   const int p = blockIdx.x * 256 + threadIdx.x;
@@ -156,11 +191,11 @@
     if constexpr (Acc::kMeasureOnly) {
       if (p >= P) break;
     }
-    const size_t o = ((size_t)n * 2 * K + 2 * t) * P + p;
-    const Pos s = tap_pos(g, py, px, t, offset[o], offset[o + P]);
+    const Tap a = tap_operands<RAW>(offset, mask, bias, n, t, p, K, P);
+    const Pos s = tap_pos(g, py, px, t, a.oh, a.ow);
     const Bil q = bil(s.h, s.w, g.H, g.W);
     if (!q.in) continue;
-    const float m = mask[((size_t)n * K + t) * P + p];
+    const float m = a.m;
     for (int c = 0; c < nc; ++c) {
       const float gv = gc[(size_t)c * KP + (size_t)t * P] * m;
       if (gv == 0.f) continue;
@@ -172,20 +207,20 @@
 
 struct Entry { int src; float w; };
 
-template <bool FILL>
-__global__ __launch_bounds__(256) void dcn_revmap_kernel(const float* __restrict__ offset,
-                                                         const float* __restrict__ mask, int* __restrict__ cursor,
+template <bool FILL, bool RAW>
+__global__ __launch_bounds__(256) void dcn_revmap_kernel(const float* __restrict__ offset, const float* __restrict__ mask,
+                                                         const float* __restrict__ bias, int* __restrict__ cursor,
                                                          Entry* __restrict__ rec, Conv g) {
   const int P = g.Ho * g.Wo, K = g.kh * g.kw, HW = g.H * g.W;
   const int p = blockIdx.x * 256 + threadIdx.x;
   if (p >= P) return;
   const int t = blockIdx.y, n = blockIdx.z;
   const int py = p / g.Wo, px = p % g.Wo;
-  const size_t o = ((size_t)n * 2 * K + 2 * t) * P + p;
-  const Pos s = tap_pos(g, py, px, t, offset[o], offset[o + P]);
+  const Tap a = tap_operands<RAW>(offset, mask, bias, n, t, p, K, P);
+  const Pos s = tap_pos(g, py, px, t, a.oh, a.ow);
   const Bil q = bil(s.h, s.w, g.H, g.W);
   if (!q.in) return;
-  const float m = FILL ? mask[((size_t)n * K + t) * P + p] : 0.f;
+  const float m = FILL ? a.m : 0.f;
   int* cur = cursor + ((size_t)n * K + t) * HW;
   const int src = t * P + p;
   for_corners(q, g.W, [&](int pix, float w) {
@@ -221,17 +256,17 @@
                                                                 const int* __restrict__ first,
                                                                 const int* __restrict__ last,
                                                                 const Entry* __restrict__ rec,
-                                                                float* __restrict__ grad_x, Conv g) {
+                                                                float* grad_x, const float* base, Conv g) {
   const int P = g.Ho * g.Wo, K = g.kh * g.kw, HW = g.H * g.W;
   const int pix = blockIdx.x * 256 + threadIdx.x;
   if (pix >= HW) return;
   const int n = blockIdx.z, c0 = blockIdx.y * kGC;
-  float acc[kGC];
-#pragma unroll
-  for (int c = 0; c < kGC; ++c) acc[c] = 0.f;
   const size_t KP = (size_t)K * P;
   const float* gc = grad_cols + ((size_t)n * g.C + c0) * KP;
   const int nc = min(kGC, g.C - c0);
+  float acc[kGC];
+#pragma unroll
+  for (int c = 0; c < kGC; ++c) acc[c] = (base && c < nc) ? base[((size_t)n * g.C + c0 + c) * HW + pix] : 0.f;
   for (int t = 0; t < K; ++t) {
     const size_t bin = ((size_t)n * K + t) * HW + pix;
     const int e0 = first[bin], e1 = last[bin];
@@ -281,7 +316,7 @@
 
 __global__ __launch_bounds__(256) void dcn_col2im_gather_lds_kernel(
     const float* __restrict__ grad_cols, const int* __restrict__ first, const int* __restrict__ last,
-    const Entry* __restrict__ rec, float* __restrict__ grad_x, Conv g, int tiles_x, int tiles_y, int nimg, float inv_wo) {
+    const Entry* __restrict__ rec, float* grad_x, const float* base, Conv g, int tiles_x, int tiles_y, int nimg, float inv_wo) {
   __shared__ __attribute__((aligned(16))) float s_gc[kGLC * kGWS];
   constexpr int K = 9;
   const int P = g.Ho * g.Wo, HW = g.H * g.W;
@@ -296,9 +331,12 @@
   const float* gc = grad_cols + ((size_t)n * g.C + c0) * KP;
   float acc[kGRY][kGLC];
 #pragma unroll
-  for (int k = 0; k < kGRY; ++k)
-#pragma unroll
-    for (int c = 0; c < kGLC; ++c) acc[k][c] = 0.f;
+  for (int k = 0; k < kGRY; ++k) {
+    const int dy = tyi * kGTH + ry + 8 * k;
+    const bool in = base && dx < g.W && dy < g.H;
+#pragma unroll
+    for (int c = 0; c < kGLC; ++c) acc[k][c] = (in && c < nc) ? base[((size_t)n * g.C + c0 + c) * HW + dy * g.W + dx] : 0.f;
+  }
   for (int t = 0; t < K; ++t) {
     const int i = t / 3, j = t - i * 3;
     const int wy0 = tyi * kGTH + g.pad - i - kGHalo - 1, wx0 = txi * kGTW + g.pad - j - kGHalo - 1;
@@ -360,19 +398,20 @@
 
 int g_dcn_variant = 1;
 
-template <bool PAIR>
+template <bool PAIR, bool RAW>
 __device__ __forceinline__ void col2im_coord_body(const float* __restrict__ grad_cols, const float* __restrict__ x,
                                                   const float* __restrict__ offset, const float* __restrict__ mask,
-                                                  float* __restrict__ grad_offset, float* __restrict__ grad_mask,
-                                                  const Conv& g) {
+                                                  const float* __restrict__ bias, float* __restrict__ grad_offset,
+                                                  float* __restrict__ grad_mask, const Conv& g) {
   const int P = g.Ho * g.Wo, K = g.kh * g.kw;
   const int p = blockIdx.x * 256 + threadIdx.x;
   if (p >= P) return;
   const int t = blockIdx.y, n = blockIdx.z;
   const int py = p / g.Wo, px = p % g.Wo;
-  const size_t o = ((size_t)n * 2 * K + 2 * t) * P + p;
-  const Pos s = tap_pos(g, py, px, t, offset[o], offset[o + P]);
-  const float m = mask[((size_t)n * K + t) * P + p];
+  const size_t o = tap_index<RAW>::off(n, t, p, K, P);
+  const Tap op = tap_operands<RAW>(offset, mask, bias, n, t, p, K, P);
+  const Pos s = tap_pos(g, py, px, t, op.oh, op.ow);
+  const float m = op.m;
   const Bil q = bil(s.h, s.w, g.H, g.W);
   float gh = 0.f, gw = 0.f, gm = 0.f;
   if (q.in) {
@@ -420,18 +459,25 @@
   }
   grad_offset[o] = gh * m;
   grad_offset[o + P] = gw * m;
-  grad_mask[((size_t)n * K + t) * P + p] = gm;
+  if constexpr (RAW) grad_offset[tap_index<RAW>::msk(n, t, p, K, P)] = gm * (m * (1.f - m));
+  else grad_mask[tap_index<RAW>::msk(n, t, p, K, P)] = gm;
 }
 
 __global__ __launch_bounds__(256) void dcn_col2im_coord_kernel(
     const float* __restrict__ grad_cols, const float* __restrict__ x, const float* __restrict__ offset,
     const float* __restrict__ mask, float* __restrict__ grad_offset, float* __restrict__ grad_mask, Conv g) {
-  col2im_coord_body<true>(grad_cols, x, offset, mask, grad_offset, grad_mask, g);
+  col2im_coord_body<true, false>(grad_cols, x, offset, mask, nullptr, grad_offset, grad_mask, g);
 }
 __global__ __launch_bounds__(256) void dcn_col2im_coord_1col_kernel(
     const float* __restrict__ grad_cols, const float* __restrict__ x, const float* __restrict__ offset,
     const float* __restrict__ mask, float* __restrict__ grad_offset, float* __restrict__ grad_mask, Conv g) {
-  col2im_coord_body<false>(grad_cols, x, offset, mask, grad_offset, grad_mask, g);
+  col2im_coord_body<false, false>(grad_cols, x, offset, mask, nullptr, grad_offset, grad_mask, g);
+}
+template <bool PAIR>
+__global__ __launch_bounds__(256) void dcn_col2im_coord_raw_kernel(
+    const float* __restrict__ grad_cols, const float* __restrict__ x, const float* __restrict__ raw,
+    const float* __restrict__ bias, float* __restrict__ grad_raw, Conv g) {
+  col2im_coord_body<PAIR, true>(grad_cols, x, raw, nullptr, bias, grad_raw, nullptr, g);
 }
 
 inline bool dcn_bad(int N, const Conv& g) {
@@ -439,69 +485,54 @@
          g.kw <= 0 || g.stride <= 0 || g.dil <= 0 || g.pad < 0;
 }
 
-}
-
-extern "C" {
-
-int vidar_dcn_set_variant(int variant) {
-  const int prev = g_dcn_variant;
-  if (variant >= 0 && variant <= 1) g_dcn_variant = variant;
-  return prev;
-}
-
-int vidar_dcn_im2col_f32(const float* x, const float* offset, const float* mask, float* cols, int N,
-                         int C, int H, int W, int Ho, int Wo, int kh, int kw, int stride, int pad,
-                         int dil, void* stream) {
-  VIDAR_ENTER();
-  Conv g{C, H, W, Ho, Wo, kh, kw, stride, pad, dil};
+template <bool RAW>
+int im2col_launch(const float* x, const float* offset, const float* mask, const float* bias, float* cols, int N, const Conv& g,
+                  hipStream_t s) {
   if (dcn_bad(N, g)) return VIDAR_ERR_BAD_ARG;
   if (N == 0) return 0;
-  if (kh * kw > kMaxTaps) return VIDAR_ERR_BAD_ARG;
-  hipLaunchKernelGGL(W >= 2 ? dcn_im2col_pair_kernel : dcn_im2col_kernel,
-                     dim3(xcd_plane_grid((Ho * Wo + 255) / 256, ((C + kCP - 1) / kCP) * N)), dim3(256), 0, (hipStream_t)stream,
-                     x, offset, mask, cols, g, N);
+  if (g.kh * g.kw > kMaxTaps) return VIDAR_ERR_BAD_ARG;
+  const dim3 grid(xcd_plane_grid((g.Ho * g.Wo + 255) / 256, ((g.C + kCP - 1) / kCP) * N));
+  if constexpr (RAW)
+    hipLaunchKernelGGL(g.W >= 2 ? dcn_im2col_raw_kernel<true> : dcn_im2col_raw_kernel<false>, grid, dim3(256), 0, s, x, offset,
+                       bias, cols, g, N);
+  else
+    hipLaunchKernelGGL(g.W >= 2 ? dcn_im2col_pair_kernel : dcn_im2col_kernel, grid, dim3(256), 0, s, x, offset, mask, cols, g, N);
   return vidar_last_error();
 }
 
-size_t vidar_dcn_col2im_workspace_bytes(int N, int H, int W, int Ho, int Wo, int kh, int kw) {
+size_t col2im_workspace_bytes(int N, int H, int W, int Ho, int Wo, int kh, int kw) {
   if (N <= 0 || H <= 0 || W <= 0 || Ho <= 0 || Wo <= 0 || kh <= 0 || kw <= 0) return 0;
   const size_t hw = (size_t)N * kh * kw * H * W, ent = (size_t)N * kh * kw * Ho * Wo * 4;
   if (ent >= (1ull << 31)) return 0;
   return sizeof(int) * 2 * hw + sizeof(Entry) * ent;
 }
 
-int vidar_dcn_col2im_det_workspace_bytes(int N, int C, int H, int W, int64_t* bytes) {
-  if (N < 0 || C < 0 || H < 0 || W < 0 || !bytes) return VIDAR_ERR_BAD_ARG;
-  *bytes = (int64_t)det_workspace_bytes((size_t)N * C * H * W);
-  return 0;
-}
-
-int vidar_dcn_col2im_f32(const float* grad_cols, const float* x, const float* offset,
-                         const float* mask, float* grad_x, float* grad_offset, float* grad_mask,
-                         int N, int C, int H, int W, int Ho, int Wo, int kh, int kw, int stride,
-                         int pad, int dil, void* workspace, size_t workspace_bytes, void* stream) {
-  VIDAR_ENTER();
-  Conv g{C, H, W, Ho, Wo, kh, kw, stride, pad, dil};
+template <bool RAW>
+int col2im_launch(const float* grad_cols, const float* x, const float* offset, const float* mask, const float* bias,
+                  float* grad_x, const float* base, float* grad_offset, float* grad_mask, int N, const Conv& g,
+                  void* workspace, size_t workspace_bytes, hipStream_t s) {
   if (dcn_bad(N, g)) return VIDAR_ERR_BAD_ARG;
-  hipStream_t s = (hipStream_t)stream;
   if (N == 0) return 0;
-  if (kh * kw > kMaxTaps) return VIDAR_ERR_BAD_ARG;
+  if (g.kh * g.kw > kMaxTaps) return VIDAR_ERR_BAD_ARG;
+  const int C = g.C, H = g.H, W = g.W, Ho = g.Ho, Wo = g.Wo, kh = g.kh, kw = g.kw;
   const int P = Ho * Wo, K = kh * kw, HW = H * W;
-  if (det_mode()) {
+  if (!grad_x) {
+  } else if (det_mode()) {
+    if constexpr (RAW) return VIDAR_ERR_BAD_ARG;
     const dim3 grid((P + 255) / 256, (C + kCG - 1) / kCG, N);
     const int rc = det_scatter(
         grad_x, nullptr, (size_t)N * C * HW, 0, (uint64_t)N * C * K * P * 4, false, workspace, workspace_bytes, s,
         [&](uint32_t* word, uint32_t*) {
-          hipLaunchKernelGGL((dcn_col2im_kernel<det::AccMeasure, det::AccMeasure::Param>), grid, dim3(256), 0, s, grad_cols, offset, mask, grad_x, g,
-                             det::AccMeasure::Param{word});
+          hipLaunchKernelGGL((dcn_col2im_kernel<det::AccMeasure, false, det::AccMeasure::Param>), grid, dim3(256), 0, s, grad_cols, offset, mask,
+                             bias, grad_x, g, det::AccMeasure::Param{word});
         },
         [&](long long* acc, long long*, const uint32_t* word, const uint32_t*, int h) {
-          hipLaunchKernelGGL((dcn_col2im_kernel<det::AccFixed, det::AccFixed::Param>), grid, dim3(256), 0, s, grad_cols, offset, mask, grad_x, g,
-                             det::AccFixed::Param{acc, word, h});
+          hipLaunchKernelGGL((dcn_col2im_kernel<det::AccFixed, false, det::AccFixed::Param>), grid, dim3(256), 0, s, grad_cols, offset, mask,
+                             bias, grad_x, g, det::AccFixed::Param{acc, word, h});
         });
     if (rc != 0) return rc;
   } else if (workspace) {
-    const size_t need = vidar_dcn_col2im_workspace_bytes(N, H, W, Ho, Wo, kh, kw);
+    const size_t need = col2im_workspace_bytes(N, H, W, Ho, Wo, kh, kw);
     if (need == 0 || workspace_bytes < need) return VIDAR_ERR_BAD_ARG;
     int* cursor = (int*)workspace;
     int* first = cursor + (size_t)N * K * HW;
@@ -509,26 +540,89 @@
     hipError_t e = hipMemsetAsync(cursor, 0, sizeof(int) * (size_t)N * K * HW, s);
     if (e != hipSuccess) return (int)e;
     const dim3 rgrid((P + 255) / 256, K, N);
-    hipLaunchKernelGGL(dcn_revmap_kernel<false>, rgrid, dim3(256), 0, s, offset, mask, cursor, rec, g);
+    hipLaunchKernelGGL((dcn_revmap_kernel<false, RAW>), rgrid, dim3(256), 0, s, offset, mask, bias, cursor, rec, g);
     hipLaunchKernelGGL(dcn_revmap_scan_kernel, dim3(N * K), dim3(1024), 0, s, cursor, first, HW, P * 4);
-    hipLaunchKernelGGL(dcn_revmap_kernel<true>, rgrid, dim3(256), 0, s, offset, mask, cursor, rec, g);
-    if ((g_dcn_variant & 1) && kh == 3 && kw == 3 && stride == 1 && dil == 1 && Ho == H && Wo == W) {
+    hipLaunchKernelGGL((dcn_revmap_kernel<true, RAW>), rgrid, dim3(256), 0, s, offset, mask, bias, cursor, rec, g);
+    if ((g_dcn_variant & 1) && kh == 3 && kw == 3 && g.stride == 1 && g.dil == 1 && Ho == H && Wo == W) {
       const int tiles_x = (W + kGTW - 1) / kGTW, tiles_y = (H + kGTH - 1) / kGTH;
       hipLaunchKernelGGL(dcn_col2im_gather_lds_kernel, dim3(xcd_plane_grid(tiles_x * tiles_y, ((C + kGLC - 1) / kGLC) * N)), dim3(256), 0,
-                         s, grad_cols, first, cursor, rec, grad_x, g, tiles_x, tiles_y, N, 1.0f / (float)Wo);
+                         s, grad_cols, first, cursor, rec, grad_x, base, g, tiles_x, tiles_y, N, 1.0f / (float)Wo);
     } else {
       hipLaunchKernelGGL(dcn_col2im_gather_kernel, dim3((HW + 255) / 256, (C + kGC - 1) / kGC, N), dim3(256), 0, s,
-                         grad_cols, first, cursor, rec, grad_x, g);
+                         grad_cols, first, cursor, rec, grad_x, base, g);
     }
   } else {
-    hipError_t e = hipMemsetAsync(grad_x, 0, sizeof(float) * (size_t)N * C * H * W, s);
+    const size_t bytes = sizeof(float) * (size_t)N * C * H * W;
+    hipError_t e = hipSuccess;
+    if (!base) e = hipMemsetAsync(grad_x, 0, bytes, s);
+    else if (base != grad_x) e = hipMemcpyAsync(grad_x, base, bytes, hipMemcpyDeviceToDevice, s);
     if (e != hipSuccess) return (int)e;
-    hipLaunchKernelGGL(dcn_col2im_kernel<det::AccAtomic>, dim3((P + 255) / 256, (C + kCG - 1) / kCG, N), dim3(256), 0, s, grad_cols,
-                       offset, mask, grad_x, g);
-  }
-  hipLaunchKernelGGL(W >= 2 ? dcn_col2im_coord_kernel : dcn_col2im_coord_1col_kernel, dim3((P + 255) / 256, K, N), dim3(256), 0,
-                     s, grad_cols, x, offset, mask, grad_offset, grad_mask, g);
+    hipLaunchKernelGGL((dcn_col2im_kernel<det::AccAtomic, RAW>), dim3((P + 255) / 256, (C + kCG - 1) / kCG, N), dim3(256), 0, s, grad_cols,
+                       offset, mask, bias, grad_x, g);
+  }
+  if (grad_offset) {
+    const dim3 grid((P + 255) / 256, K, N);
+    if constexpr (RAW)
+      hipLaunchKernelGGL(W >= 2 ? dcn_col2im_coord_raw_kernel<true> : dcn_col2im_coord_raw_kernel<false>, grid, dim3(256), 0, s,
+                         grad_cols, x, offset, bias, grad_offset, g);
+    else
+      hipLaunchKernelGGL(W >= 2 ? dcn_col2im_coord_kernel : dcn_col2im_coord_1col_kernel, grid, dim3(256), 0, s, grad_cols, x,
+                         offset, mask, grad_offset, grad_mask, g);
+  }
   return vidar_last_error();
 }
 
 }
+
+extern "C" {
+
+int vidar_dcn_set_variant(int variant) {
+  const int prev = g_dcn_variant;
+  if (variant >= 0 && variant <= 1) g_dcn_variant = variant;
+  return prev;
+}
+
+int vidar_dcn_im2col_f32(const float* x, const float* offset, const float* mask, float* cols, int N,
+                         int C, int H, int W, int Ho, int Wo, int kh, int kw, int stride, int pad,
+                         int dil, void* stream) {
+  VIDAR_ENTER();
+  return im2col_launch<false>(x, offset, mask, nullptr, cols, N, Conv{C, H, W, Ho, Wo, kh, kw, stride, pad, dil}, (hipStream_t)stream);
+}
+
+int vidar_dcn_im2col_raw_f32(const float* x, const float* raw, const float* raw_bias, float* cols, int N,
+                             int C, int H, int W, int Ho, int Wo, int kh, int kw, int stride, int pad,
+                             int dil, void* stream) {
+  VIDAR_ENTER();
+  return im2col_launch<true>(x, raw, nullptr, raw_bias, cols, N, Conv{C, H, W, Ho, Wo, kh, kw, stride, pad, dil}, (hipStream_t)stream);
+}
+
+size_t vidar_dcn_col2im_workspace_bytes(int N, int H, int W, int Ho, int Wo, int kh, int kw) {
+  return col2im_workspace_bytes(N, H, W, Ho, Wo, kh, kw);
+}
+
+int vidar_dcn_col2im_det_workspace_bytes(int N, int C, int H, int W, int64_t* bytes) {
+  if (N < 0 || C < 0 || H < 0 || W < 0 || !bytes) return VIDAR_ERR_BAD_ARG;
+  *bytes = (int64_t)det_workspace_bytes((size_t)N * C * H * W);
+  return 0;
+}
+
+int vidar_dcn_col2im_f32(const float* grad_cols, const float* x, const float* offset,
+                         const float* mask, float* grad_x, float* grad_offset, float* grad_mask,
+                         int N, int C, int H, int W, int Ho, int Wo, int kh, int kw, int stride,
+                         int pad, int dil, void* workspace, size_t workspace_bytes, void* stream) {
+  VIDAR_ENTER();
+  return col2im_launch<false>(grad_cols, x, offset, mask, nullptr, grad_x, nullptr, grad_offset, grad_mask, N,
+                              Conv{C, H, W, Ho, Wo, kh, kw, stride, pad, dil}, workspace, workspace_bytes, (hipStream_t)stream);
+}
+
+int vidar_dcn_col2im_raw_f32(const float* grad_cols, const float* x, const float* raw, const float* raw_bias,
+                             float* grad_x, const float* grad_x_base, float* grad_raw, int N, int C, int H, int W,
+                             int Ho, int Wo, int kh, int kw, int stride, int pad, int dil, void* workspace,
+                             size_t workspace_bytes, void* stream) {
+  VIDAR_ENTER();
+  if (det_mode()) return VIDAR_ERR_BAD_ARG;
+  return col2im_launch<true>(grad_cols, x, raw, nullptr, raw_bias, grad_x, grad_x_base, grad_raw, nullptr, N,
+                             Conv{C, H, W, Ho, Wo, kh, kw, stride, pad, dil}, workspace, workspace_bytes, (hipStream_t)stream);
+}
+
+}
diff --git a/vidar_amd/plugin/backbones.py b/vidar_amd/plugin/backbones.py
--- a/vidar_amd/plugin/backbones.py
+++ b/vidar_amd/plugin/backbones.py
@@ -35,6 +35,40 @@
     return gx, goff, gm
 
 
+def _dcn_out_size(H, W, kh, kw, stride, pad, dil):
+    return (H + 2 * pad - dil * (kh - 1) - 1) // stride + 1, (W + 2 * pad - dil * (kw - 1) - 1) // stride + 1
+
+
+def _dcn_product(weight, bias, cols, gemm_mode, scale, shift, relu):
+    N, Cout = cols.shape[0], weight.shape[0]
+    fused = scale is not None
+    if gemm_mode == "lib":
+        assert not fused
+        out = torch.bmm(weight.reshape(1, Cout, -1).expand(N, -1, -1), cols)
+        if bias is not None:
+            out = out + bias.view(1, -1, 1)
+        return out
+    sh = shift
+    if bias is not None:
+        sh = bias.float() if not fused else (shift + bias.float() * scale)
+    return G.conv_forward(weight.reshape(Cout, -1), cols, scale, sh, None, relu, G.precision_of(gemm_mode))
+
+
+def _dcn_product_backward(grad_out, weight, cols, scale, y, gemm_mode, relu, need_weight):
+    N, Cout = cols.shape[0], weight.shape[0]
+    go = grad_out.float().contiguous().view(N, Cout, -1)
+    if scale is not None:
+        go = _affine_act_backward(go, y if relu else go, scale, relu, False)[0]
+    if gemm_mode == "lib":
+        grad_weight = torch.bmm(go, cols.transpose(1, 2)).sum(0).reshape(weight.shape)
+        grad_cols = torch.bmm(weight.reshape(1, Cout, -1).transpose(1, 2).expand(N, -1, -1), go)
+    else:
+        prec = G.precision_of(gemm_mode)
+        grad_weight = G.conv_grad_weight(go, cols, prec).reshape(weight.shape) if need_weight else None
+        grad_cols = G.conv_grad_input(weight.reshape(Cout, -1), go, prec)
+    return go, grad_weight, grad_cols
+
+
 class _ModulatedDeformConv(Function):
 
     @staticmethod
@@ -43,23 +77,13 @@
         x, offset, mask = x.float().contiguous(), offset.float().contiguous(), mask.float().contiguous()
         N, C, H, W = x.shape
         Cout, _, kh, kw = weight.shape
-        Ho = (H + 2 * pad - dil * (kh - 1) - 1) // stride + 1
-        Wo = (W + 2 * pad - dil * (kw - 1) - 1) // stride + 1
+        Ho, Wo = _dcn_out_size(H, W, kh, kw, stride, pad, dil)
         cols = torch.empty((N, C * kh * kw, Ho * Wo), device=x.device)
         with TIMER.span("dcn_im2col", 4 * (x.numel() + offset.numel() + mask.numel() + cols.numel())):
             check(lib().vidar_dcn_im2col_f32(ptr(x), ptr(offset), ptr(mask), ptr(cols), N, C, H, W, Ho,
                                              Wo, kh, kw, stride, pad, dil, stream_of(x)), "dcn_im2col")
         fused = scale is not None
-        if gemm_mode == "lib":
-            assert not fused
-            out = torch.bmm(weight.reshape(1, Cout, -1).expand(N, -1, -1), cols)
-            if bias is not None:
-                out = out + bias.view(1, -1, 1)
-        else:
-            sh = shift
-            if bias is not None:
-                sh = bias.float() if not fused else (shift + bias.float() * scale)
-            out = G.conv_forward(weight.reshape(Cout, -1), cols, scale, sh, None, relu, G.precision_of(gemm_mode))
+        out = _dcn_product(weight, bias, cols, gemm_mode, scale, shift, relu)
         ctx.save_for_backward(x, offset, mask, weight, cols, scale, out if (fused and relu) else None)
         ctx.cfg = (stride, pad, dil, Ho, Wo, bias is not None, gemm_mode, fused, relu)
         return out.view(N, Cout, Ho, Wo)
@@ -71,16 +95,8 @@
         stride, pad, dil, Ho, Wo, has_bias, gemm_mode, fused, relu = ctx.cfg
         N, C, H, W = x.shape
         Cout, _, kh, kw = weight.shape
-        go = grad_out.float().contiguous().view(N, Cout, Ho * Wo)
-        if fused:
-            go = _affine_act_backward(go, y if relu else go, scale, relu, False)[0]
-        if gemm_mode == "lib":
-            grad_weight = torch.bmm(go, cols.transpose(1, 2)).sum(0).reshape(weight.shape)
-            grad_cols = torch.bmm(weight.reshape(1, Cout, -1).transpose(1, 2).expand(N, -1, -1), go)
-        else:
-            prec = G.precision_of(gemm_mode)
-            grad_weight = G.conv_grad_weight(go, cols, prec).reshape(weight.shape) if ctx.needs_input_grad[3] else None
-            grad_cols = G.conv_grad_input(weight.reshape(Cout, -1), go, prec)
+        go, grad_weight, grad_cols = _dcn_product_backward(grad_out, weight, cols, scale, y, gemm_mode, relu,
+                                                           ctx.needs_input_grad[3])
         gx, goff, gm = dcn_col2im(grad_cols, x, offset, mask, kh, kw, stride, pad, dil, Ho, Wo)
         return (gx, goff, gm, grad_weight, (go.sum((0, 2)) if has_bias else None), None, None, None, None, None, None,
                 None)
@@ -99,19 +115,24 @@
 _CONV_OFFSET_OWN = os.environ.get("VIDAR_CONV_OFFSET", "lib") == "own"
 
 
+def _conv3x3_few(x, w, bias):
+    N, C, H, W = x.shape
+    Cout = w.shape[0]
+    out = torch.empty((N, Cout, H, W), device=x.device, dtype=torch.float32)
+    ws, ws_ptr, ws_bytes = workspace(lib().vidar_conv3x3_few_workspace_bytes, C, like=x)
+    with TIMER.span("conv3x3_few", 4 * (x.numel() + out.numel())):
+        check(lib().vidar_conv3x3_few_f32(ptr(x), ptr(w), ptr(bias), ptr(out), N, C, H, W, Cout, ws_ptr, ws_bytes,
+                                          stream_of(x)), "conv3x3_few")
+    return out
+
+
 class _Conv3x3Few(Function):
 
     @staticmethod
     def forward(ctx, x, weight, bias):
         x = x.contiguous()
         w = weight.contiguous()
-        N, C, H, W = x.shape
-        Cout = w.shape[0]
-        out = torch.empty((N, Cout, H, W), device=x.device, dtype=torch.float32)
-        ws, ws_ptr, ws_bytes = workspace(lib().vidar_conv3x3_few_workspace_bytes, C, like=x)
-        with TIMER.span("conv3x3_few", 4 * (x.numel() + out.numel())):
-            check(lib().vidar_conv3x3_few_f32(ptr(x), ptr(w), ptr(bias), ptr(out), N, C, H, W, Cout, ws_ptr, ws_bytes,
-                                              stream_of(x)), "conv3x3_few")
+        out = _conv3x3_few(x, w, bias)
         ctx.save_for_backward(x, w)
         ctx.has_bias = bias is not None
         return out
@@ -132,6 +153,75 @@
             and conv.kernel_size == (3, 3) and conv.stride == (1, 1) and conv.padding == (1, 1) and conv.dilation == (1, 1)
             and conv.groups == 1 and conv.padding_mode == "zeros" and conv.out_channels <= 32 and conv.in_channels % 8 == 0
             and x.shape[3] <= 191 and x.shape[2] * x.shape[3] < (1 << 30) and x.numel() > 0)
+
+
+_DCN_PACK = os.environ.get("VIDAR_DCN_PACK", "1") != "0"
+
+
+def dcn_im2col_raw(x, raw, raw_bias, kh, kw, stride, pad, dil):
+    N, C, H, W = x.shape
+    Ho, Wo = raw.shape[2:]
+    cols = torch.empty((N, C * kh * kw, Ho * Wo), device=x.device)
+    with TIMER.span("dcn_im2col", 4 * (x.numel() + raw.numel() + cols.numel())):
+        check(lib().vidar_dcn_im2col_raw_f32(ptr(x), ptr(raw), ptr(raw_bias), ptr(cols), N, C, H, W, Ho, Wo, kh, kw,
+                                             stride, pad, dil, stream_of(x)), "dcn_im2col_raw")
+    return cols
+
+
+def dcn_col2im_raw(grad_cols, x, raw, raw_bias, kh, kw, stride, pad, dil, grad_x=None, grad_x_base=None, grad_raw=None,
+                   gather=True):
+    N, C, H, W = x.shape
+    Ho, Wo = raw.shape[2:]
+    ws, ws_ptr, nbytes = workspace(lib().vidar_dcn_col2im_workspace_bytes, N, H, W, Ho, Wo, kh, kw, like=x) \
+        if (gather and grad_x is not None) else (None, None, 0)
+    with TIMER.span("dcn_col2im", 4 * ((3 * x.numel() if grad_x is not None else 0)
+                                       + (x.numel() + 2 * raw.numel() if grad_raw is not None else 0) + grad_cols.numel())):
+        check(lib().vidar_dcn_col2im_raw_f32(ptr(grad_cols), ptr(x), ptr(raw), ptr(raw_bias), ptr(grad_x), ptr(grad_x_base),
+                                             ptr(grad_raw), N, C, H, W, Ho, Wo, kh, kw, stride, pad, dil, ws_ptr, nbytes,
+                                             stream_of(x)), "dcn_col2im_raw")
+
+
+class _DeformConvPack(Function):
+
+    @staticmethod
+    def forward(ctx, x, w_off, b_off, weight, bias, stride, pad, dil, gemm_mode, scale, shift, relu, own_offset):
+        x, w_off = x.contiguous(), w_off.contiguous()
+        b_off = b_off.contiguous() if b_off is not None else None
+        N, C, H, W = x.shape
+        Cout, _, kh, kw = weight.shape
+        if own_offset:
+            raw = _conv3x3_few(x, w_off, None)
+        else:
+            raw = F.conv2d(x, w_off, None, stride, pad, dil).contiguous()
+        cols = dcn_im2col_raw(x, raw, b_off, kh, kw, stride, pad, dil)
+        out = _dcn_product(weight, bias, cols, gemm_mode, scale, shift, relu)
+        if any(ctx.needs_input_grad):
+            fused = scale is not None
+            ctx.save_for_backward(x, raw, w_off, b_off, weight, cols, scale, out if (fused and relu) else None)
+            ctx.cfg = (stride, pad, dil, bias is not None, gemm_mode, relu)
+        return out.view(N, Cout, *raw.shape[2:])
+
+    @staticmethod
+    @once_differentiable
+    def backward(ctx, grad_out):
+        x, raw, w_off, b_off, weight, cols, scale, y = ctx.saved_tensors
+        stride, pad, dil, has_bias, gemm_mode, relu = ctx.cfg
+        kh, kw = weight.shape[2:]
+        need_x, need_woff, need_boff, need_w = ctx.needs_input_grad[:4]
+        need_boff = need_boff and b_off is not None
+        go, grad_weight, grad_cols = _dcn_product_backward(grad_out, weight, cols, scale, y, gemm_mode, relu, need_w)
+        gx = gw_off = gb_off = None
+        if need_x or need_woff or need_boff:
+            grad_raw = torch.empty_like(raw)
+            dcn_col2im_raw(grad_cols, x, raw, b_off, kh, kw, stride, pad, dil, grad_raw=grad_raw)
+            gx, gw_off, gb_off = torch.ops.aten.convolution_backward(
+                grad_raw, x, w_off, [w_off.shape[0]] if b_off is not None else None, [stride] * 2, [pad] * 2, [dil] * 2, False,
+                [0, 0], 1, [need_x, need_woff, need_boff])
+        if need_x:
+            gx = gx.contiguous()
+            dcn_col2im_raw(grad_cols, x, raw, b_off, kh, kw, stride, pad, dil, grad_x=gx, grad_x_base=gx)
+        return (gx, gw_off, gb_off, grad_weight, (go.sum((0, 2)) if has_bias else None), None, None, None, None, None, None,
+                None, None)
 
 
 class ModulatedDeformConv2dPack(nn.Module):
@@ -151,7 +241,22 @@
         nn.init.zeros_(self.conv_offset.weight)
         nn.init.zeros_(self.conv_offset.bias)
 
+    def _one_node_ok(self, x):
+        co = self.conv_offset
+        return (_DCN_PACK and x.is_cuda and x.dim() == 4 and x.numel() > 0 and not torch.is_autocast_enabled()
+                and all(t is None or t.dtype == torch.float32 for t in (x, self.weight, self.bias, co.weight, co.bias))
+                and self.k * self.k <= 9 and not deterministic.enabled())
+
     def forward(self, x, bn=None, relu=False):
+        if self._one_node_ok(x):
+            m = G.mode() if G.own_kernels() else "lib"
+            scale = shift = None
+            if bn is not None:
+                assert m != "lib"
+                scale, shift = bn._scale_shift()
+            co = self.conv_offset
+            return _DeformConvPack.apply(x, co.weight, co.bias, self.weight, self.bias, int(self.stride), int(self.padding),
+                                         int(self.dilation), m, scale, shift, bool(relu), conv3x3_few_ok(co, x))
         if conv3x3_few_ok(self.conv_offset, x):
             out = _Conv3x3Few.apply(x, self.conv_offset.weight, self.conv_offset.bias)
         else:
```

After: 2.947, median of 6. About the same (+0.4%).
